# whwu95/MVFNet

Hardware: AMD Instinct MI355X
Metric: clips/sec (fwd+bwd) MVFNet-R50 8x8 224^2 (higher is better)
Workload: dtype bf16; 1 GPU; MVFNet-ResNet50 8x8, 32 clips/GPU of 8x3x224x224, bf16, train step: fwd (batch-stat BN) + loss + bwd + clip + SGD-nesterov; all through the HIP C ABI (stem + 16 bottlenecks + MVF + TSN head); clips_per_gpu=32, frames_per_clip=8, parallelism=dp1: replicas, one flat gradient all-reduce per step

## Files before the change

include/mvfnet_hip.h:

```cpp
#ifndef MVFNET_HIP_H
#define MVFNET_HIP_H

#include <stddef.h>
#include <stdint.h>

#ifdef __cplusplus
extern "C" {
#endif

#define MVF_ABI_VERSION 2

enum { MVF_OK = 0, MVF_EINVAL = -1, MVF_ESHAPE = -2, MVF_EWS = -3, MVF_EHIP = -4, MVF_EUNSUPPORTED = -5 };
enum { MVF_F32 = 0, MVF_BF16 = 1 };
enum { MVF_NCHW = 0, MVF_NHWC = 1 };
enum { MVF_VIEW_T = 1, MVF_VIEW_H = 2, MVF_VIEW_W = 4 };

int mvf_abi_version(void);
const char* mvf_last_error(void);

typedef struct {
    int32_t nt, c, h, w;
    int32_t n_segment;
    int32_t cs;
    int32_t mode;
// ... 14 lines not shown
                  const float* w_t, const float* w_h, const float* w_w,
                  const float* gamma, const float* beta, float eps, float momentum,
                  float* running_mean, float* running_var, float* save_mean, float* save_invstd,
                  void* ws, size_t ws_bytes, void* stream);

size_t mvf_bwd_workspace_bytes(const mvf_desc_t* d);
int mvf_bwd(const mvf_desc_t* d, const void* g, const void* x,
            const float* w_t, const float* w_h, const float* w_w,
            const float* gamma, const float* beta, const float* mean, const float* invstd, int training,
            void* dx, float* dw_t, float* dw_h, float* dw_w, float* dgamma, float* dbeta,
            void* ws, size_t ws_bytes, void* stream);


typedef struct {
    int32_t n, h, w;
    int32_t cin, cout;
    int32_t kh, kw, stride, pad;
    int32_t ho, wo;
    int32_t x_pix_stride;
    int32_t dtype;
    int32_t relu;
    int32_t split_c;
    int32_t x2_pix_stride;
    int32_t in_dil;
    int32_t res_c0;
    int32_t x_c0;
} mvf_conv_desc_t;

int mvf_conv2d_nhwc_fwd(const mvf_conv_desc_t* d, const void* x, const void* x2, const void* w_packed,
                        const float* bias, const void* residual, void* y, void* stream);
size_t mvf_conv2d_workspace_bytes(const mvf_conv_desc_t* d);
int mvf_conv2d_nhwc_fwd_ws(const mvf_conv_desc_t* d, const void* x, const void* x2, const void* w_packed,
                           const float* bias, const void* residual, void* y, void* ws, size_t ws_bytes, void* stream);
int mvf_conv2d_nhwc_fwd_mvf(const mvf_conv_desc_t* d, const void* x, const void* w_packed, const float* bias, const float* mvf_coef,
                            int cs, int n_segment, int act, void* y, void* ws, size_t ws_bytes, void* stream);
int mvf_conv2d_nhwc_fwd_bnapply(const mvf_conv_desc_t* d, const void* x, const void* x2, const void* w_packed, const float* bn_scale,
                                const float* bn_shift, const void* residual, const float* res_scale, const float* res_shift, void* out,
                                unsigned char* sign_bits, void* ws, size_t ws_bytes, void* stream);
int mvf_conv2d_nhwc_fwd_bnbwd_sums(const mvf_conv_desc_t* d, const void* x, const void* x2, const void* w_packed, const void* g,
                                   const unsigned char* sign_bits, const float* bn_mean, const float* bn_invstd, float* sums_part, void* ws,
                                   size_t ws_bytes, void* stream);
int mvf_conv2d_nhwc_fwd_bnbwd_apply(const mvf_conv_desc_t* d, const void* x, const void* x2, const void* w_packed, const void* g,
                                    const unsigned char* sign_bits, const float* bn_gamma, const float* bn_mean, const float* bn_invstd,
                                    const float* dgamma, const float* dbeta, void* dz, void* ws, size_t ws_bytes, void* stream);
int mvf_conv2d_nhwc_fwd_resmask(const mvf_conv_desc_t* d, const void* x, const void* x2, const void* w_packed,
                                const float* bias, const void* residual, const unsigned char* res_sign_bits, void* y,
                                void* ws, size_t ws_bytes, void* stream);
int mvf_conv2d_nhwc_fwd_resmask_gate(const mvf_conv_desc_t* d, const void* x, const void* x2, const void* w_packed, const float* bias,
                                     const void* residual, const unsigned char* res_sign_bits, const unsigned char* out_gate_bits, void* y,
                                     void* ws, size_t ws_bytes, void* stream);
int mvf_conv2d_nhwc_fwd_resmask_gate_colsums(const mvf_conv_desc_t* d, const void* x, const void* x2, const void* w_packed, const void* residual,
                                             const unsigned char* res_sign_bits, const unsigned char* out_gate_bits, void* y, float* sums_part, void* ws,
                                             size_t ws_bytes, void* stream);
int mvf_conv2d_nhwc_dgrad_bnsums(const mvf_conv_desc_t* d, const void* dz, const void* w_packed_dgrad, void* y, const void* bn_z,
                                 const float* bn_mean, const float* bn_invstd, const float* bn_scale, const float* bn_shift,
                                 float* sums_part, void* ws, size_t ws_bytes, void* stream);
int mvf_bn_bwd_finalize(const float* sums_part, int nblk, int c, float* dgamma, float* dbeta, void* stream);
int mvf_conv2d_stats_rows(const mvf_conv_desc_t* d);
int mvf_conv2d_nhwc_fwd_stats(const mvf_conv_desc_t* d, const void* x, const void* x2, const void* w_packed, void* y,
                              float* stats_part, const float* stats_shift, void* ws, size_t ws_bytes, void* stream);

enum {
    MVF_CONV_FAM_NONE = 0,
    MVF_CONV_FAM_REG = 1,
    MVF_CONV_FAM_X3 = 2,
    MVF_CONV_FAM_LDS_DMA = 3,
    MVF_CONV_FAM_T256_2B = 4,
    MVF_CONV_FAM_T256_P4 = 5,
    MVF_CONV_FAM_DBUF = 6,
    MVF_CONV_FAM_DBUF_PF2 = 7,
    MVF_CONV_FAM_STREAMK = 8,
    MVF_CONV_FAM_GENERIC = 9,
    MVF_CONV_FAM_MVF_LOADER = 10,
    MVF_CONV_FAM_STEM_DIRECT = 11,
    MVF_CONV_FAM_PW_SUMS = 12,
    MVF_CONV_FAM_C3X3_C64 = 13
};
typedef struct {
    int32_t family;
    int32_t epi_asked;
    int32_t epi_run;
    int32_t pointwise;
    int32_t buffers;
    int32_t tile_m, tile_n;
    int32_t dtype;
    int32_t k_chunks;
    int32_t half_k;
    int32_t launches;
} mvf_conv_launch_info_t;
int mvf_conv2d_last_launch(mvf_conv_launch_info_t* out);

int mvf_pack_conv_weight(const float* w_oihw, int cout, int cin, int kh, int kw, int kw_pad, int cin_pad,
                         const float* scale, void* w_packed, int dtype, void* stream);
int mvf_bn_fold(const float* gamma, const float* beta, const float* mean, const float* var, float eps, int c,
                float* scale, float* shift, void* stream);

int mvf_stem_prep(const float* x_nchw, int n, int c, int h, int w, int pad, int wp, void* out, int dtype, void* stream);

int mvf_frames_prep_u8(const unsigned char* frames_hwc, int n, int hs, int ws, const int* window, int h, int w,
                       const float* mean3, const float* std3, int to_rgb, int div_255, int pad, int wp, void* out_stem,
                       float* out_nchw, int dtype, void* stream);
int mvf_frames_resample_u8(const unsigned char* frames_hwc, int n, int hs, int ws, const int* rows, int h, int w,
                           const float* mean3, const float* std3, int to_rgb, int div_255, int pad, int wp, void* out_stem,
                           float* out_nchw, int dtype, void* stream);
int mvf_frames_resample_color_u8(const unsigned char* frames_hwc, int n, int hs, int ws, const int* rows, const float* color, int h, int w,
                                 const float* mean3, const float* std3, int to_rgb, int div_255, int pad, int wp, void* out_stem,
// ... 164 lines not shown
int mvf_conv2d_nhwc_wgrad(const mvf_conv_desc_t* d, const void* dz, const void* x, const void* x2, int kw_real,
                          int cin_real, int kw_packed, int cin_packed, float* dw_oihw, void* ws, size_t ws_bytes,
                          void* stream);
int mvf_conv2d_nhwc_wgrad_wgs(const mvf_conv_desc_t* d, const void* dz, const void* x, const void* x2, int kw_real,
                              int cin_real, int kw_packed, int cin_packed, float* dw_oihw, void* ws, size_t ws_bytes, int wgs, void* stream);
enum {
    MVF_WGRAD_FAM_NONE = 0,
    MVF_WGRAD_FAM_F32_REG = 1,
    MVF_WGRAD_FAM_F32_DMA = 2,
    MVF_WGRAD_FAM_X3 = 3,
    MVF_WGRAD_FAM_BF16_WIDEN = 4,
    MVF_WGRAD_FAM_BF16_REG = 5,
    MVF_WGRAD_FAM_BF16_DMA2 = 6,
    MVF_WGRAD_FAM_BF16_PIPE = 7,
    MVF_WGRAD_FAM_T256_2B = 8,
    MVF_WGRAD_FAM_T256_P4 = 9,
    MVF_WGRAD_FAM_C3X3_C64 = 10,
    MVF_WGRAD_FAM_STEM = 11
};
typedef struct {
    int32_t family;
    int32_t stages;
    int32_t tile_co, tile_k;
    int32_t dtype;
    int32_t nsplit;
    int32_t rows_per_split;
    int32_t xcd_rr;
    int32_t split_operand;
    int32_t gram;
    int32_t wgs_target;
    int32_t launches;
} mvf_wgrad_launch_info_t;
int mvf_conv2d_wgrad_last_launch(mvf_wgrad_launch_info_t* out);
typedef struct {
    const float* w;
    void* out;
    int cout, cin, kh, kw, kw_pad, cin_pad;
    int kind, first_block;
} mvf_pack_job_t;
int mvf_pack_conv_weights_batched(const mvf_pack_job_t* jobs_dev, int njobs, int total_blocks, int dtype, void* stream);

int mvf_pack_conv_weight_dgrad(const float* w_oihw, int cout, int cin, int kh, int kw, void* w_packed, int dtype,
                               void* stream);
int mvf_nhwc_stencil(const mvf_desc_t* d, const void* x, int x_c, void* out, int out_c, const float* w_t,
                     const float* w_h, const float* w_w, const float* scale, const float* shift, int flip,
                     const void* addend, int addend_c, const unsigned char* addend_sign_bits, void* stream);
int mvf_nhwc_stencil_gate(const mvf_desc_t* d, const void* x, int x_c, void* out, int out_c, const float* w_t,
                          const float* w_h, const float* w_w, const float* scale, const float* shift, int flip,
                          const void* addend, int addend_c, const unsigned char* addend_sign_bits,
                          const unsigned char* out_gate_bits, void* stream);
int mvf_nhwc_stencil_gate_colsums(const mvf_desc_t* d, const void* x, int x_c, void* out, int out_c, const float* w_t, const float* w_h,
                                  const float* w_w, int flip, const void* addend, int addend_c, const unsigned char* addend_sign_bits,
                                  const unsigned char* out_gate_bits, float* sums_part, void* stream);
int mvf_nhwc_stencil_stats_rows(const mvf_desc_t* d, int x_c, int out_c);
int mvf_nhwc_stencil_tile_plan(const mvf_desc_t* d, int x_c, int out_c, int* rows_per_band, int* chan_per_wg);
int mvf_nhwc_stencil_stats(const mvf_desc_t* d, const void* x, int x_c, void* out, int out_c, const float* w_t, const float* w_h,
                           const float* w_w, float* stats_part, const float* stats_shift, void* stream);
size_t mvf_nhwc_tapgrad_workspace_bytes(const mvf_desc_t* d);
int mvf_nhwc_tapgrad(const mvf_desc_t* d, const void* x, int x_c, const void* dy, int dy_c, float* dw_t, float* dw_h,
                     float* dw_w, void* ws, size_t ws_bytes, void* stream);
enum {
    MVF_STENCIL_KERNEL_NONE = 0,
    MVF_STENCIL_KERNEL_WALK1 = 1,
    MVF_STENCIL_KERNEL_WALK4 = 2,
    MVF_STENCIL_KERNEL_CHUNKED = 3,
    MVF_STENCIL_KERNEL_LDS = 4
};
enum {
    MVF_STENCIL_FLIP = 1, MVF_STENCIL_HSWISH = 2, MVF_STENCIL_ADDEND = 4, MVF_STENCIL_ADDEND_BITS = 8, MVF_STENCIL_OUT_GATE = 16,
    MVF_STENCIL_STATS = 32,
    MVF_STENCIL_TAIL_COPY = 64
};
typedef struct {
    int32_t kernel;
    int32_t dtype;
    int32_t frames_per_chunk;
    int32_t rows_per_band, chan_per_wg;
    int32_t bands;
    int32_t pixels_per_wg;
    int32_t grid_x, grid_y;
    int32_t partial_rows;
    int32_t flags;
    int32_t launches;
} mvf_stencil_launch_info_t;
int mvf_nhwc_stencil_last_launch(mvf_stencil_launch_info_t* out);
enum {
    MVF_TAPGRAD_KERNEL_NONE = 0,
    MVF_TAPGRAD_KERNEL_ROWS = 1,
    MVF_TAPGRAD_KERNEL_BANDS = 2
};
typedef struct {
    int32_t kernel;
    int32_t dtype;
    int32_t nblk;
    int32_t rows_per_blk;
    int32_t cgp;
    int32_t grid_y;
    int32_t launches;
} mvf_tapgrad_launch_info_t;
int mvf_nhwc_tapgrad_last_launch(mvf_tapgrad_launch_info_t* out);
size_t mvf_sgd_workspace_bytes(long n);
int mvf_sgd_nesterov_step(float* params, const float* grads, float* momentum_buf, long n, float grad_scale, float max_norm,
                          float lr, float momentum, float weight_decay, int first_step, float* norm_out, void* ws,
                          size_t ws_bytes, void* stream);
typedef struct mvf_sgd_segment {
    long long first;
// ... 82 lines not shown
```

mvfnet_amd/_lib.py:

```python
import ctypes as C
import os

import torch

_HERE = os.path.dirname(os.path.abspath(__file__))
LIB_PATH = os.environ.get("MVF_LIB_PATH") or os.path.join(_HERE, "libmvfnet_hip.so")

MVF_F32, MVF_BF16 = 0, 1
MVF_NCHW, MVF_NHWC = 0, 1
VIEW_T, VIEW_H, VIEW_W = 1, 2, 4
MODE_BITS = {"T": 1, "TH": 3, "THW": 7}
METRICS_ROWS, METRICS_BAD_LABEL, METRICS_NAN_ROWS, METRICS_HITS, METRICS_MAX_K, METRICS_CONFUSION = 0, 1, 2, 8, 8, 16
MULTILABEL_SLOTS, MULTILABEL_NAN_ROWS, MULTILABEL_OVERFLOW, MULTILABEL_SEEN, MULTILABEL_STATE_WORDS = 0, 1, 2, 3, 8
ERRNAMES = {-1: "MVF_EINVAL", -2: "MVF_ESHAPE", -3: "MVF_EWS", -4: "MVF_EHIP", -5: "MVF_EUNSUPPORTED"}


class MvfDesc(C.Structure):
    _fields_ = [("nt", C.c_int32), ("c", C.c_int32), ("h", C.c_int32), ("w", C.c_int32), ("n_segment", C.c_int32),
                ("cs", C.c_int32), ("mode", C.c_int32), ("layout", C.c_int32), ("dtype", C.c_int32)]


class ConvDesc(C.Structure):
    _fields_ = [("n", C.c_int32), ("h", C.c_int32), ("w", C.c_int32), ("cin", C.c_int32), ("cout", C.c_int32),
                ("kh", C.c_int32), ("kw", C.c_int32), ("stride", C.c_int32), ("pad", C.c_int32),
# ... 84 lines not shown
    _fields_ = [("ptr", C.c_void_p), ("first", C.c_long)]


def _load():
    if not os.path.exists(LIB_PATH):
        raise ImportError(
            "mvfnet_amd: %s not found. Build it with `python -m mvfnet_amd.build` (needs hipcc, "
            "--offload-arch=gfx950). There is no CPU or PyTorch fallback for the hot path." % LIB_PATH)
    lib = C.CDLL(LIB_PATH)
    vp, fp, sz, i32, f32 = C.c_void_p, C.c_void_p, C.c_size_t, C.c_int, C.c_float
    dp = C.POINTER(MvfDesc)
    lib.mvf_abi_version.restype = i32
    lib.mvf_abi_version.argtypes = []
    lib.mvf_last_error.restype = C.c_char_p
    lib.mvf_last_error.argtypes = []
    lib.mvf_fwd_infer.restype = i32
    lib.mvf_fwd_infer.argtypes = [dp, vp, vp, fp, fp, fp, fp, fp, vp]
    lib.mvf_fwd_train_workspace_bytes.restype = sz
    lib.mvf_fwd_train_workspace_bytes.argtypes = [dp]
    lib.mvf_fwd_train.restype = i32
    lib.mvf_fwd_train.argtypes = [dp, vp, vp, fp, fp, fp, fp, fp, f32, f32, fp, fp, fp, fp, vp, sz, vp]
    lib.mvf_bwd_workspace_bytes.restype = sz
    lib.mvf_bwd_workspace_bytes.argtypes = [dp]
    lib.mvf_bwd.restype = i32
    lib.mvf_bwd.argtypes = [dp, vp, vp, fp, fp, fp, fp, fp, fp, fp, i32, vp, fp, fp, fp, fp, fp, vp, sz, vp]
    lib.mvf_fwd_infer_slice.restype = i32
    lib.mvf_fwd_infer_slice.argtypes = [dp, vp, vp, fp, fp, fp, fp, fp, vp]
    cp = C.POINTER(ConvDesc)
    lib.mvf_conv2d_nhwc_fwd.restype = i32
    lib.mvf_conv2d_nhwc_fwd.argtypes = [cp, vp, vp, vp, fp, vp, vp, vp]
    lib.mvf_conv2d_workspace_bytes.restype = sz
    lib.mvf_conv2d_workspace_bytes.argtypes = [cp]
    lib.mvf_conv2d_nhwc_fwd_ws.restype = i32
    lib.mvf_conv2d_nhwc_fwd_ws.argtypes = [cp, vp, vp, vp, fp, vp, vp, vp, sz, vp]
    lib.mvf_conv2d_nhwc_dgrad_bnsums.restype = i32
    lib.mvf_conv2d_nhwc_dgrad_bnsums.argtypes = [cp, vp, vp, vp, vp, fp, fp, fp, fp, fp, vp, sz, vp]
    lib.mvf_bn_bwd_finalize.restype = i32
    lib.mvf_bn_bwd_finalize.argtypes = [fp, i32, i32, fp, fp, vp]
    lib.mvf_conv2d_nhwc_fwd_bnapply.restype = i32
    lib.mvf_conv2d_nhwc_fwd_bnapply.argtypes = [cp, vp, vp, vp, fp, fp, vp, fp, fp, vp, vp, vp, sz, vp]
    lib.mvf_conv2d_nhwc_fwd_bnbwd_sums.restype = i32
    lib.mvf_conv2d_nhwc_fwd_bnbwd_sums.argtypes = [cp, vp, vp, vp, vp, vp, fp, fp, fp, vp, sz, vp]
    lib.mvf_conv2d_nhwc_fwd_bnbwd_apply.restype = i32
    lib.mvf_conv2d_nhwc_fwd_bnbwd_apply.argtypes = [cp, vp, vp, vp, vp, vp, fp, fp, fp, fp, fp, vp, vp, sz, vp]
    lib.mvf_conv2d_nhwc_fwd_resmask.restype = i32
    lib.mvf_conv2d_nhwc_fwd_resmask.argtypes = [cp, vp, vp, vp, fp, vp, vp, vp, vp, sz, vp]
    i64_ = C.c_long
    lib.mvf_conv2d_nhwc_fwd_resmask_gate.restype = i32
    lib.mvf_conv2d_nhwc_fwd_resmask_gate.argtypes = [cp, vp, vp, vp, fp, vp, vp, vp, vp, vp, sz, vp]
    lib.mvf_conv2d_nhwc_fwd_resmask_gate_colsums.restype = i32
    lib.mvf_conv2d_nhwc_fwd_resmask_gate_colsums.argtypes = [cp, vp, vp, vp, vp, vp, vp, vp, fp, vp, sz, vp]
    lib.mvf_nhwc_stencil_gate_colsums.restype = i32
    lib.mvf_nhwc_stencil_gate_colsums.argtypes = [dp, vp, i32, vp, i32, fp, fp, fp, i32, vp, i32, vp, vp, fp, vp]
    lib.mvf_conv2d_nhwc_dgrad_bnsums_split.restype = i32
    lib.mvf_conv2d_nhwc_dgrad_bnsums_split.argtypes = [cp, vp, vp, vp, fp, vp, vp, fp, fp, fp, fp, fp, vp, sz, vp]
    lib.mvf_bn_bwd_dzfree_prep.restype = i32
    lib.mvf_bn_bwd_dzfree_prep.argtypes = [vp, i32, i32, fp, fp, fp, fp, fp, i64_, vp, fp, i32, vp]
    lib.mvf_bn_bwd_dzfree_wgrad.restype = i32
    lib.mvf_bn_bwd_dzfree_wgrad.argtypes = [fp, vp, fp, fp, fp, fp, fp, fp, fp, i64_, i32, i32, i32, vp]
    lib.mvf_bn_bwd_dzfree_sums.restype = i32
    lib.mvf_bn_bwd_dzfree_sums.argtypes = [fp, vp, i32, i32, fp, fp, fp, i32, i32, fp, i32, fp, fp, i32, vp]
    lib.mvf_nhwc_stencil_stats_rows.restype = i32
    lib.mvf_nhwc_stencil_stats_rows.argtypes = [dp, i32, i32]
    lib.mvf_nhwc_stencil_tile_plan.restype = i32
    lib.mvf_nhwc_stencil_tile_plan.argtypes = [dp, i32, i32, C.POINTER(C.c_int), C.POINTER(C.c_int)]
    lib.mvf_nhwc_stencil_stats.restype = i32
    lib.mvf_nhwc_stencil_stats.argtypes = [dp, vp, i32, vp, i32, fp, fp, fp, fp, fp, vp]
    lib.mvf_nhwc_stencil_gate.restype = i32
    lib.mvf_nhwc_stencil_gate.argtypes = [dp, vp, i32, vp, i32, fp, fp, fp, fp, fp, i32, vp, i32, vp, vp, vp]
    lib.mvf_conv2d_stats_rows.restype = i32
    lib.mvf_conv2d_stats_rows.argtypes = [cp]
    lib.mvf_conv2d_nhwc_fwd_stats.restype = i32
    lib.mvf_conv2d_nhwc_fwd_stats.argtypes = [cp, vp, vp, vp, vp, fp, fp, vp, sz, vp]
    lib.mvf_conv2d_last_launch.restype = i32
    lib.mvf_conv2d_last_launch.argtypes = [C.POINTER(ConvLaunchInfo)]
    lib.mvf_pack_conv_weight.restype = i32
    lib.mvf_pack_conv_weight.argtypes = [fp, i32, i32, i32, i32, i32, i32, fp, vp, i32, vp]
    lib.mvf_pack_conv_weights_batched.restype = i32
    lib.mvf_pack_conv_weights_batched.argtypes = [vp, i32, i32, i32, vp]
    lib.mvf_bn_fold.restype = i32
    lib.mvf_bn_fold.argtypes = [fp, fp, fp, fp, f32, i32, fp, fp, vp]
    lib.mvf_stem_prep.restype = i32
    lib.mvf_stem_prep.argtypes = [fp, i32, i32, i32, i32, i32, i32, vp, i32, vp]
    lib.mvf_frames_prep_u8.restype = i32
    lib.mvf_frames_prep_u8.argtypes = [vp, i32, i32, i32, vp, i32, i32, C.POINTER(C.c_float), C.POINTER(C.c_float),
                                       i32, i32, i32, i32, vp, vp, i32, vp]
    lib.mvf_frames_resample_u8.restype = i32
    lib.mvf_frames_resample_u8.argtypes = [vp, i32, i32, i32, vp, i32, i32, C.POINTER(C.c_float), C.POINTER(C.c_float),
                                           i32, i32, i32, i32, vp, vp, i32, vp]
    lib.mvf_frames_resample_color_u8.restype = i32
    lib.mvf_frames_resample_color_u8.argtypes = [vp, i32, i32, i32, vp, vp, i32, i32, C.POINTER(C.c_float), C.POINTER(C.c_float),
                                                 i32, i32, i32, i32, vp, vp, i32, vp]
    lib.mvf_frames_gather_resample_u8.restype = i32
    lib.mvf_frames_gather_resample_u8.argtypes = [vp, i32, i32, i32, vp, i32, vp, vp, i32, i32, C.POINTER(C.c_float), C.POINTER(C.c_float),
                                                  i32, i32, i32, i32, vp, vp, i32, vp]
    lib.mvf_frames_yuv420_gather_resample_u8.restype = i32
    lib.mvf_frames_yuv420_gather_resample_u8.argtypes = [vp, i32, i32, i32, i32, i32, i32, i32, vp, i32, vp, vp, i32, i32, C.POINTER(C.c_float),
                                                         C.POINTER(C.c_float), i32, i32, i32, i32, vp, vp, i32, vp]
    lib.mvf_frames_addressed_resample_u8.restype = i32
    lib.mvf_frames_addressed_resample_u8.argtypes = [vp, C.c_longlong, i32, i32, i32, i32, vp, vp, vp, i32, i32, C.POINTER(C.c_float), C.POINTER(C.c_float),
                                                     i32, i32, i32, i32, vp, vp, i32, vp]
    lib.mvf_maxpool3x3s2_nhwc.restype = i32
    lib.mvf_maxpool3x3s2_nhwc.argtypes = [vp, i32, i32, i32, i32, vp, i32, vp]
    lib.mvf_head_pool_fc.restype = i32
    lib.mvf_head_pool_fc.argtypes = [vp, i32, i32, i32, i32, fp, fp, i32, fp, fp, i32, vp]
    lib.mvf_average_clip.restype = i32
# ... 185 lines not shown
```

mvfnet_amd/csrc/conv_nhwc.hip:

```cpp
#include <algorithm>
#include <type_traits>
#include <stdlib.h>
#include <string.h>

#include "common.h"

namespace {

constexpr int kThreads = 256;
constexpr int kPitch = 144;
constexpr int kBM = 128;

typedef float f32x16 __attribute__((ext_vector_type(16)));
typedef short bf16x8 __attribute__((ext_vector_type(8)));

struct ConvArgs {
    const char* x;
    const char* x2;
    const char* w;
    const char* res;
    const float* bias;
    char* y;
    int N, H, W, Cin, Cout, KH, KW, stride, pad, Ho, Wo;
    int xps, split_c, x2ps, relu;
    int res_c0;
    const unsigned char* res_mask;
    const unsigned char* out_gate;
    int x_c0;
    int mask_lds;
    int prio;
    int dil;
    int pad_w;
    int w_kh0, w_kw0, w_ts, w_kwfull;
    int o_s, o_ph, o_pw, o_hfull, o_wfull;
    float* stats_part;
    int stats_rows;
    const float* stats_shift;
    const char* bn_z;
    const float *bn_mean, *bn_invstd, *bn_scale, *bn_shift;
    const float *ap_scale, *ap_shift, *ap_rscale, *ap_rshift;
    unsigned char* ap_bits;
    const float *bw_gamma, *bw_dgamma, *bw_dbeta;
    int bw_mode;
    const float* mvf_coef;
    int mvf_cs, mvf_T, mvf_act;
    unsigned fd_t_mul, fd_t_shr;
    int M;
    int cpt;
    int nchunks;
    long wK;
    int tiles_m, tiles_n;
    unsigned fd_hw_mul, fd_hw_shr, fd_w_mul, fd_w_shr;
};

template <typename ET>
struct TT;
template <>
struct TT<float> {
    static constexpr int ESZ = 4, UE = 4, CE = 32;
};
template <>
struct TT<bf16_t> {
    static constexpr int ESZ = 2, UE = 8, CE = 64;
};

thread_local mvf_conv_launch_info_t t_last_launch = {};
inline void note_launch(int family, int epi_asked, int epi_run, bool pw, int buffers, int bm, int bn, int esz, int nchunks, bool half_k = false) {
    mvf_conv_launch_info_t& r = t_last_launch;
    const int launches = r.launches + 1;
    r = mvf_conv_launch_info_t{family, epi_asked, epi_run, pw ? 1 : 0, buffers, bm, bn, esz == 4 ? MVF_F32 : MVF_BF16, nchunks, half_k ? 1 : 0, launches};
}

__device__ __forceinline__ int fd_div(int n, unsigned mul, unsigned shr) { return (int)((__umulhi((unsigned)n, mul) + (unsigned)n) >> shr); }
inline void fd_make(unsigned d, unsigned& mul, unsigned& shr) {
    unsigned l = 0;
    while ((1ull << l) < d) ++l;
    mul = (unsigned)((((1ull << l) - d) << 32) / d + 1);
    shr = l;
// ... 714 lines not shown
    }

#ifdef MVF_CONV_ABLATE
    if (a.prio & 16) return;
#endif
    if (mode == SEG_PRODUCE) {
        float* slot = sk.ws + (long)g_self * (BM * BN);
#pragma unroll
        for (int i = 0; i < TM; ++i)
#pragma unroll
            for (int j = 0; j < TN; ++j)
#pragma unroll
                for (int r = 0; r < 16; ++r) slot[((i * TN + j) * 16 + r) * NT + tid] = acc[i][j][r];
        asm volatile("s_waitcnt vmcnt(0)" ::: "memory");
        __syncthreads();
        if (tid == 0) {
            __builtin_amdgcn_fence(__ATOMIC_RELEASE, "agent");
            asm volatile("s_waitcnt vmcnt(0)" ::: "memory");
            __hip_atomic_store(sk.flags + g_self, 1u, __ATOMIC_RELAXED, __HIP_MEMORY_SCOPE_AGENT);
        }
        return;
    }
    if (mode == SEG_FINISH) {
        for (int g = g_first; g < g_self; ++g) {
            if (tid == 0) {
                unsigned spins = 0;
                while (__hip_atomic_load(sk.flags + g, __ATOMIC_RELAXED, __HIP_MEMORY_SCOPE_AGENT) == 0u) {
                    __builtin_amdgcn_s_sleep(4);
                    if (++spins > (1u << 26)) {
                        __hip_atomic_store(sk.err, 1u, __ATOMIC_RELAXED, __HIP_MEMORY_SCOPE_AGENT);
                        break;
                    }
                }
                __builtin_amdgcn_fence(__ATOMIC_ACQUIRE, "agent");
            }
            __syncthreads();
            const float* slot = sk.ws + (long)g * (BM * BN);
#pragma unroll
            for (int i = 0; i < TM; ++i)
#pragma unroll
                for (int j = 0; j < TN; ++j)
#pragma unroll
                    for (int r = 0; r < 16; ++r) acc[i][j][r] += slot[((i * TN + j) * 16 + r) * NT + tid];
        }
    }

    const bool e_bias = EPI == 0 ? a.bias != nullptr : (EPI == 4 || EPI == 5 || (EPI == 6 && a.bias != nullptr));
    const bool e_res = EPI == 0 ? a.res != nullptr : (EPI == 3 || EPI == 5 || EPI == 8 || EPI == 9 || EPI == 10 || EPI == 12);
    constexpr bool e_bw = EPI == 9 || EPI == 10;
    const bool e_relu = EPI == 0 ? a.relu != 0 : (EPI == 4 || EPI == 5);
    constexpr bool e_apply = EPI == 8;
    const bool e_stats = EPI == 0 ? a.stats_part != nullptr : (EPI == 1 || EPI == 12);
    constexpr bool e_bnb = EPI == 6;
    const bool e_scatter = (EPI == 0 || EPI == 6) && a.o_s > 0;
    constexpr int CP = BN * 4 + 16;
    constexpr int NH = (LOWK || GLDS) ? 2 : 1;
    constexpr int HR = BM / NH;
    static_assert(HR * CP <= kSmem, "C tile (or half) must fit in the A/B LDS buffers");
    static_assert(HR % 32 == 0, "half split follows the MFMA row tiles");
    constexpr int PPT = BM / kBM;
    constexpr int HPP = NH / PPT;
    static_assert(NH % PPT == 0 && HPP >= 1, "a statistics partial covers whole epilogue passes");
    constexpr int TPR = BN / 4, RPP = NT / TPR;
    const int cq = tid % TPR, r0 = tid / TPR;
    const int col = n0 + cq * 4;
    ET* y = reinterpret_cast<ET*>(a.y);
    const ET* res = reinterpret_cast<const ET*>(a.res);
    float4 bv = make_float4(0.f, 0.f, 0.f, 0.f);
    if (e_bias && col < a.Cout) bv = *reinterpret_cast<const float4*>(a.bias + col);
    float4 st1 = make_float4(0.f, 0.f, 0.f, 0.f), st2 = st1, kk = st1;
    if (e_stats && a.stats_shift && col < a.Cout) kk = *reinterpret_cast<const float4*>(a.stats_shift + col);
    float4 ap_s = st1, ap_b = st1, ap_rs = make_float4(1.f, 1.f, 1.f, 1.f), ap_rb = st1;
    if (e_apply && col < a.Cout) {
        ap_s = *reinterpret_cast<const float4*>(a.ap_scale + col); ap_b = *reinterpret_cast<const float4*>(a.ap_shift + col);
        if (a.ap_rscale) { ap_rs = *reinterpret_cast<const float4*>(a.ap_rscale + col); ap_rb = *reinterpret_cast<const float4*>(a.ap_rshift + col); }
    }
    float4 b_mu = st1, b_rs = st1, b_sc = st1, b_sh = st1;
    if (e_bnb && col < a.Cout) {
        b_mu = *reinterpret_cast<const float4*>(a.bn_mean + col); b_rs = *reinterpret_cast<const float4*>(a.bn_invstd + col);
        b_sc = *reinterpret_cast<const float4*>(a.bn_scale + col); b_sh = *reinterpret_cast<const float4*>(a.bn_shift + col);
    }
    float4 w_a = st1, w_d0 = st1, w_kx = st1;
    if (e_bw && col < a.Cout) {
        b_mu = *reinterpret_cast<const float4*>(a.bn_mean + col); b_rs = *reinterpret_cast<const float4*>(a.bn_invstd + col);
        if constexpr (EPI == 9) {
            const float inv_m = 1.0f / (float)a.M;
            const float4 ga = *reinterpret_cast<const float4*>(a.bw_gamma + col), dg = *reinterpret_cast<const float4*>(a.bw_dgamma + col),
                         db = *reinterpret_cast<const float4*>(a.bw_dbeta + col);
            w_a = make_float4(ga.x * b_rs.x, ga.y * b_rs.y, ga.z * b_rs.z, ga.w * b_rs.w);
            w_d0 = make_float4(db.x * inv_m, db.y * inv_m, db.z * inv_m, db.w * inv_m);
            w_kx = make_float4(b_rs.x * dg.x * inv_m, b_rs.y * dg.y * inv_m, b_rs.z * dg.z * inv_m, b_rs.w * dg.w * inv_m);
        }
    }
    typedef unsigned u32x2 __attribute__((ext_vector_type(2)));
    const int eimg0 = fd_div(m0, a.fd_hw_mul, a.fd_hw_shr);
    __amdgpu_buffer_rsrc_t rs_y, rs_res;
    {
        const long total = (e_scatter ? (long)a.N * a.o_hfull * a.o_wfull : (long)a.M) * a.Cout * ESZ;
        const long base = (e_scatter ? (long)eimg0 * a.o_hfull * a.o_wfull : (long)m0) * a.Cout * ESZ;
        const long left = total - base;
        const unsigned nrec = (unsigned)(left < 0x7ffffff0L ? left : 0x7ffffff0L);
        rs_y = __builtin_amdgcn_make_buffer_rsrc((void*)(a.y + base), 0, a.y ? nrec : 0u, 0x00020000);
        rs_res = __builtin_amdgcn_make_buffer_rsrc((void*)(e_res ? a.res + base : (e_bnb ? a.bn_z + base : a.y + base)), 0, nrec, 0x00020000);
    }
    const __amdgpu_buffer_rsrc_t rs_mask = __builtin_amdgcn_make_buffer_rsrc(
        (void*)(a.res_mask ? a.res_mask + (long)m0 * (a.Cout / 4) : (const unsigned char*)a.y), 0,
        (unsigned)min((long)(a.M - m0) * (a.Cout / 4), 0x7ffffff0L), 0x00020000);
    const __amdgpu_buffer_rsrc_t rs_gate = __builtin_amdgcn_make_buffer_rsrc(
        (void*)(a.out_gate ? a.out_gate + (long)m0 * (a.Cout / 4) : (const unsigned char*)a.y), 0,
        (unsigned)min((long)(a.M - m0) * (a.Cout / 4), 0x7ffffff0L), 0x00020000);
    const bool e_gate = e_res && !e_apply && !e_bw && a.out_gate != nullptr;
    (void)y; (void)res;
    constexpr int kMaskOff = HR * CP;
    constexpr int MSEG = BN / 64;
    static_assert(kMaskOff + BM * (BN / 4) <= kSmem, "mask tile must fit behind the C tile");
    const bool mask_lds = e_res && (a.res_mask || e_gate) && (a.Cout % 64 == 0) && a.mask_lds;
    if (mask_lds) {
#pragma unroll
        for (int it = tid; it < BM * MSEG; it += NT) {
            const int row = it / MSEG, seg = it - row * MSEG;
            const unsigned moff = (unsigned)(row * (a.Cout / 4) + n0 / 4 + seg * 16);
            u32x4 mv = {0x0f0f0f0fu, 0x0f0f0f0fu, 0x0f0f0f0fu, 0x0f0f0f0fu};
            if (a.res_mask) mv = __builtin_amdgcn_raw_buffer_load_b128(rs_mask, moff, 0, 0);
            if (e_gate) {
                const u32x4 gv = __builtin_amdgcn_raw_buffer_load_b128(rs_gate, moff, 0, 0);
                mv.x = (mv.x & 0x0f0f0f0fu) | ((gv.x & 0x0f0f0f0fu) << 4); mv.y = (mv.y & 0x0f0f0f0fu) | ((gv.y & 0x0f0f0f0fu) << 4);
                mv.z = (mv.z & 0x0f0f0f0fu) | ((gv.z & 0x0f0f0f0fu) << 4); mv.w = (mv.w & 0x0f0f0f0fu) | ((gv.w & 0x0f0f0f0fu) << 4);
            }
            *reinterpret_cast<uint4*>(smem + kMaskOff + row * (BN / 4) + seg * 16) = make_uint4(mv.x, mv.y, mv.z, mv.w);
        }
    }
    if constexpr (sizeof(ET) == 2 && (EPI == 1 || EPI == 2) && BM == kBM) {
        if ((a.Cout & 7) == 0) {
            constexpr int CPB = BN * 2 + 8;
            static_assert(BM * CPB <= kSmem, "bf16 C tile must fit in the A/B LDS buffers");
            constexpr int TPR8 = BN / 8, RPP8 = NT / TPR8, NPS8 = BM / RPP8;
            static_assert(2 * 2 * RPP8 * TPR8 * 16 <= kSmem, "statistics scratch");
#pragma unroll
            for (int j = 0; j < TN; ++j)
#pragma unroll
                for (int i = 0; i < TM; ++i) {
                    char* cp = smem + ((wm * TM + i) * 32 + (lane & 31)) * CPB + ((wn * TN + j) * 32 + 4 * (lane >> 5)) * 2;
#pragma unroll
                    for (int g = 0; g < 4; ++g) {
                        uint2 pk;
                        pk.x = pack_bf16x2(acc[i][j][4 * g], acc[i][j][4 * g + 1]);
                        pk.y = pack_bf16x2(acc[i][j][4 * g + 2], acc[i][j][4 * g + 3]);
                        *reinterpret_cast<uint2*>(cp + g * 16) = pk;
                    }
                }
            const int cq8 = tid % TPR8, r08 = tid / TPR8;
            const int col8 = n0 + cq8 * 8;
            const bool cok8 = col8 < a.Cout;
            float kk8[8], mu8[8], rs8[8], sc8[8], sh8[8], s1[8], s2[8];
#pragma unroll
            for (int k = 0; k < 8; ++k) { kk8[k] = mu8[k] = rs8[k] = sc8[k] = sh8[k] = s1[k] = s2[k] = 0.f; }
// ... 87 lines not shown
                    if (c4 < a.Cout && tm_i * kBM < a.M) {
                        float4 t1 = make_float4(0.f, 0.f, 0.f, 0.f), t2 = t1;
                        for (int r = 0; r < RPP8; ++r) {
                            const float4 p1 = red[((r * 2 + 0) * 2 + h) * TPR8 + cq], p2 = red[((r * 2 + 1) * 2 + h) * TPR8 + cq];
                            t1.x += p1.x; t1.y += p1.y; t1.z += p1.z; t1.w += p1.w;
                            t2.x += p2.x; t2.y += p2.y; t2.z += p2.z; t2.w += p2.w;
                        }
                        float2* p = reinterpret_cast<float2*>(a.stats_part) + (long)c4 * a.stats_rows + tm_i;
                        p[0] = make_float2(t1.x, t2.x);
                        p[a.stats_rows] = make_float2(t1.y, t2.y);
                        p[2 * (long)a.stats_rows] = make_float2(t1.z, t2.z);
                        p[3 * (long)a.stats_rows] = make_float2(t1.w, t2.w);
                    }
                }
            }
            return;
        }
    }
#pragma unroll
    for (int hf = 0; hf < NH; ++hf) {
        if (hf > 0) __syncthreads();
#pragma unroll
        for (int j = 0; j < TN; ++j)
#pragma unroll
            for (int i = 0; i < TM; ++i) {
                const int rbase = (wm * TM + i) * 32;
                if (rbase / HR != hf) continue;
                char* cp = smem + (rbase - hf * HR + (lane & 31)) * CP + ((wn * TN + j) * 32 + 4 * (lane >> 5)) * 4;
#pragma unroll
                for (int g = 0; g < 4; ++g)
                    *reinterpret_cast<float4*>(cp + g * 32) =
                        make_float4(acc[i][j][4 * g], acc[i][j][4 * g + 1], acc[i][j][4 * g + 2], acc[i][j][4 * g + 3]);
            }
        constexpr int NPS = HR / RPP;
        typedef typename std::conditional<sizeof(ET) == 2, u32x2, u32x4>::type raw_t;
        unsigned offs[NPS];
        raw_t rraw[NPS];
        {
            const int mrow0 = m0 + hf * HR + r0;
            const bool cok2 = col < a.Cout;
#pragma unroll
            for (int ps = 0; ps < NPS; ++ps) {
                const int m = mrow0 + ps * RPP;
                unsigned off;
                if (e_scatter) {
                    const int img = fd_div(m, a.fd_hw_mul, a.fd_hw_shr), rem = m - img * (a.Ho * a.Wo);
                    const int oh = fd_div(rem, a.fd_w_mul, a.fd_w_shr), ow = rem - oh * a.Wo;
                    off = (unsigned)((((img - eimg0) * a.o_hfull + oh * a.o_s + a.o_ph) * a.o_wfull + ow * a.o_s + a.o_pw) * a.Cout + col) * ESZ;
                } else {
                    off = (unsigned)((m - m0) * a.Cout + col) * ESZ;
                }
                offs[ps] = (cok2 && m < a.M) ? off : kOOB;
                if (e_res || e_bnb) {
                    const unsigned roff = (e_bnb || col >= a.res_c0) ? offs[ps] : kOOB;
                    if constexpr (sizeof(ET) == 2) rraw[ps] = __builtin_amdgcn_raw_buffer_load_b64(rs_res, roff, 0, 0);
                    else rraw[ps] = __builtin_amdgcn_raw_buffer_load_b128(rs_res, roff, 0, 0);
                }
            }
        }
        __syncthreads();
        {
            auto unpack = [](const raw_t& t) {
                if constexpr (sizeof(ET) == 2)
                    return make_float4(__uint_as_float(t.x << 16), __uint_as_float(t.x & 0xffff0000u), __uint_as_float(t.y << 16),
                                       __uint_as_float(t.y & 0xffff0000u));
                else
                    return make_float4(__uint_as_float(t.x), __uint_as_float(t.y), __uint_as_float(t.z), __uint_as_float(t.w));
            };
#pragma unroll
            for (int ps = 0; ps < NPS; ++ps) {
                const unsigned off = offs[ps];
                const bool ok = off != kOOB;
                float4 v = *reinterpret_cast<const float4*>(smem + (r0 + ps * RPP) * CP + cq * 16);
                if constexpr (e_apply) {
                    if constexpr (sizeof(ET) == 2) {
                        const unsigned p0 = pack_bf16x2(v.x, v.y), p1 = pack_bf16x2(v.z, v.w);
                        v = make_float4(__uint_as_float(p0 << 16), __uint_as_float(p0 & 0xffff0000u), __uint_as_float(p1 << 16), __uint_as_float(p1 & 0xffff0000u));
                    }
                    const float4 q = unpack(rraw[ps]);
                    float t0 = v.x * ap_s.x + ap_b.x, t1 = v.y * ap_s.y + ap_b.y, t2 = v.z * ap_s.z + ap_b.z, t3 = v.w * ap_s.w + ap_b.w;
                    t0 += q.x * ap_rs.x + ap_rb.x; t1 += q.y * ap_rs.y + ap_rb.y; t2 += q.z * ap_rs.z + ap_rb.z; t3 += q.w * ap_rs.w + ap_rb.w;
                    v = make_float4(fmaxf(t0, 0.f), fmaxf(t1, 0.f), fmaxf(t2, 0.f), fmaxf(t3, 0.f));
                    if (ok) a.ap_bits[(long)(m0 + hf * HR + r0 + ps * RPP) * (a.Cout / 4) + (col >> 2)] =
                        (unsigned char)((v.x > 0.f ? 1u : 0u) | (v.y > 0.f ? 2u : 0u) | (v.z > 0.f ? 4u : 0u) | (v.w > 0.f ? 8u : 0u));
                }
                if constexpr (e_bw) {
                    if constexpr (sizeof(ET) == 2) {
                        const unsigned p0 = pack_bf16x2(v.x, v.y), p1 = pack_bf16x2(v.z, v.w);
                        v = make_float4(__uint_as_float(p0 << 16), __uint_as_float(p0 & 0xffff0000u), __uint_as_float(p1 << 16), __uint_as_float(p1 & 0xffff0000u));
                    }
                    float4 gm = unpack(rraw[ps]);
                    const unsigned mb = mask_lds ? (unsigned)*reinterpret_cast<const unsigned char*>(smem + kMaskOff + (hf * HR + r0 + ps * RPP) * (BN / 4) + cq)
                                                 : (unsigned)__builtin_amdgcn_raw_buffer_load_b8(rs_mask, ok ? off / (4 * ESZ) : kOOB, 0, 0);
                    gm.x = (mb & 1u) ? gm.x : 0.f; gm.y = (mb & 2u) ? gm.y : 0.f; gm.z = (mb & 4u) ? gm.z : 0.f; gm.w = (mb & 8u) ? gm.w : 0.f;
                    if constexpr (EPI == 10) {
                        if (!ok) gm = make_float4(0.f, 0.f, 0.f, 0.f);
                        st1.x += gm.x; st1.y += gm.y; st1.z += gm.z; st1.w += gm.w;
                        st2.x += gm.x * ((v.x - b_mu.x) * b_rs.x); st2.y += gm.y * ((v.y - b_mu.y) * b_rs.y);
                        st2.z += gm.z * ((v.z - b_mu.z) * b_rs.z); st2.w += gm.w * ((v.w - b_mu.w) * b_rs.w);
                        continue;
                    } else {
                        v.x = w_a.x * (gm.x - w_d0.x - (v.x - b_mu.x) * w_kx.x); v.y = w_a.y * (gm.y - w_d0.y - (v.y - b_mu.y) * w_kx.y);
                        v.z = w_a.z * (gm.z - w_d0.z - (v.z - b_mu.z) * w_kx.z); v.w = w_a.w * (gm.w - w_d0.w - (v.w - b_mu.w) * w_kx.w);
                    }
                }
                if (e_bias) { v.x += bv.x; v.y += bv.y; v.z += bv.z; v.w += bv.w; }
                if (e_res && !e_apply && !e_bw) {
// ... 89 lines not shown
    SkArgs sk = {};
    conv_tile<ET, WM, WN, TM, TN, false, false, true>(a, smem, xcd_swizzle(blockIdx.x, gridDim.x), 0, a.nchunks, SEG_FULL, sk, 0, 0);
}

template <typename ET, int WM, int WN, int TM, int TN>
__global__ __launch_bounds__(kThreads) void conv_igemm_pf2_kernel(ConvArgs a) {
    extern __shared__ __attribute__((aligned(16))) char smem[];
    SkArgs sk = {};
    conv_tile<ET, WM, WN, TM, TN, false, true>(a, smem, xcd_swizzle(blockIdx.x, gridDim.x), 0, a.nchunks, SEG_FULL, sk, 0, 0);
}

template <typename ET, int WM, int WN, int TM, int TN, int EPI = 0, bool PW = false, bool MVFL = false>
__global__ __launch_bounds__(kThreads) void conv_igemm_lowk_kernel(ConvArgs a) {
    extern __shared__ __attribute__((aligned(16))) char smem[];
    SkArgs sk = {};
    conv_tile<ET, WM, WN, TM, TN, true, false, false, EPI, PW, 0, MVFL>(a, smem, xcd_swizzle(blockIdx.x, gridDim.x), 0, a.nchunks, SEG_FULL, sk, 0, 0);
}

template <int WM, int WN, int TM, int TN, int EPI = 0, bool PW = false>
__global__ __launch_bounds__(kThreads, 3) void conv_igemm_x3_kernel(ConvArgs a) {
    extern __shared__ __attribute__((aligned(16))) char smem[];
    SkArgs sk = {};
    conv_tile<float, WM, WN, TM, TN, true, false, false, EPI, PW, 0, false, false, true>(a, smem, xcd_swizzle(blockIdx.x, gridDim.x), 0, a.nchunks, SEG_FULL, sk, 0, 0);
}

template <typename ET, int WM, int WN, int TM, int TN, int EPI, int NB, bool MVFL = false, bool PW = false, bool HALFK = false>
__global__ __launch_bounds__(kThreads, (NB == 1 && !MVFL) ? 4 : 1) void conv_igemm_glds_kernel(ConvArgs a) {
    extern __shared__ __attribute__((aligned(16))) char smem[];
    SkArgs sk = {};
    conv_tile<ET, WM, WN, TM, TN, false, false, false, EPI, PW, NB, MVFL, HALFK>(a, smem, xcd_swizzle(blockIdx.x, gridDim.x), 0, a.nchunks, SEG_FULL, sk, 0, 0);
}

inline int conv_epi_spec() {
    static const int v = mvf_policy_int("conv_epi", 3);
    return v;
}

inline bool is_pointwise(const ConvArgs& a) {
    return (conv_epi_spec() & 2) && a.KH == 1 && a.KW == 1 && a.pad == 0 && a.pad_w == 0 && a.split_c == 0 && a.dil <= 1;
}

inline bool infer_like(const ConvArgs& a, int epi_spec) { return (epi_spec & 1) && a.o_s <= 0 && a.bias && a.relu && !a.stats_part; }
inline bool bnsum_epi(const ConvArgs& a) { return a.bn_z && !a.relu && !a.res; }

int conv_epi_of(const ConvArgs& a, int epi_spec) {
    const bool train_like = (epi_spec & 1) && a.o_s <= 0 && !a.bias && !a.relu;
    if (a.ap_scale) return 8;
    if (a.bw_mode == 9 || a.bw_mode == 10) return a.bw_mode;
    if (train_like && a.stats_part && !a.res && !a.bn_z) return 1;
    if (bnsum_epi(a)) return 6;
    if (train_like && !a.stats_part && !a.res) return 2;
    if (train_like && !a.stats_part && a.res) return 3;
    if (train_like && a.stats_part && a.res && a.out_gate && !a.bn_z) return 12;
    if (infer_like(a, epi_spec)) return a.res ? 5 : 4;
    return 0;
}

template <int... E, class F>
int with_epi(int epi, F&& f) {
    int rc = MVF_OK;
    const bool hit = ((epi == E ? (rc = f(std::integral_constant<int, E>{}), true) : false) || ...);
    return hit ? rc : f(std::integral_constant<int, 0>{});
}

template <typename ET, int EPI>
__global__ __launch_bounds__(512) void conv_igemm_big2_kernel(ConvArgs a) {
    extern __shared__ __attribute__((aligned(16))) char smem[];
    SkArgs sk = {};
    conv_tile<ET, 4, 2, 2, 4, false, false, false, EPI, false, 2>(a, smem, xcd_swizzle(blockIdx.x, gridDim.x), 0, a.nchunks, SEG_FULL, sk, 0, 0);
}

template <typename ET>
int launch_big2(int epi, hipStream_t st, const ConvArgs& a0) {
    ConvArgs a = a0;
    a.tiles_m = (a.M + 255) / 256;
    a.tiles_n = (a.Cout + 255) / 256;
    return with_epi<1, 2, 3, 4, 5, 6>(epi, [&](auto e) -> int {
        constexpr int lds = kGldsLds<256, 256, 2>();
        auto k = conv_igemm_big2_kernel<ET, decltype(e)::value>;
        static bool attr = false;
        if (!attr) {
            MVF_HIP_OK(hipFuncSetAttribute((const void*)k, hipFuncAttributeMaxDynamicSharedMemorySize, lds));
            attr = true;
        }
        hipLaunchKernelGGL(k, dim3(a.tiles_m * a.tiles_n), dim3(512), lds, st, a);
        note_launch(MVF_CONV_FAM_T256_2B, epi, decltype(e)::value, false, 2, 256, 256, (int)sizeof(ET), a.nchunks);
        return MVF_OK;
    });
}

template <typename ET, int EPI, bool PW>
__global__ __launch_bounds__(512) void conv_igemm_p4_kernel(ConvArgs a) {
    extern __shared__ __attribute__((aligned(16))) char smem[];
    SkArgs sk = {};
    conv_tile<ET, 2, 4, 4, 2, false, false, false, EPI, PW, 4>(a, smem, xcd_swizzle(blockIdx.x, gridDim.x), 0, a.nchunks, SEG_FULL, sk, 0, 0);
}

template <typename ET>
int launch_p4(int epi, hipStream_t st, const ConvArgs& a0) {
    if constexpr (sizeof(ET) != 2) {
        return MVF_EUNSUPPORTED;
    } else {
        ConvArgs a = a0;
        a.tiles_m = (a.M + 255) / 256;
        a.tiles_n = (a.Cout + 255) / 256;
        return with_epi<1, 2, 3, 4, 5, 6>(epi, [&](auto e) -> int {
            constexpr int EPI = decltype(e)::value, lds = kGldsLds<256, 256, 2>();
// ... 309 lines not shown
    }
    SkArgs sk;
    const long units = (long)tail * a.nchunks;
    sk.G = slots;
    sk.units_base = (int)(units / sk.G);
    sk.units_rem = (int)(units % sk.G);
    sk.tile0 = full;
    sk.ws = (float*)skh.ws;
    sk.flags = (unsigned*)((char*)skh.ws + (size_t)slots * (128 * 128 * sizeof(float)));
    sk.err = sk.flags + slots;
    MVF_HIP_OK(hipMemsetAsync(sk.flags, 0, (size_t)(slots + 1) * sizeof(unsigned), st));
    hipLaunchKernelGGL(kern_sk, dim3(sk.G), dim3(kThreads), lds, st, a, sk);
    note_launch(MVF_CONV_FAM_STREAMK, conv_epi_of(a, conv_epi_spec()), 0, false, 2, BM, BN, (int)sizeof(ET), a.nchunks);
    MVF_LAUNCH_CHECK();
    return MVF_OK;
}

}

extern "C" {

size_t mvf_conv2d_workspace_bytes(const mvf_conv_desc_t*) { return sk_ws_bytes(); }

int mvf_conv2d_last_launch(mvf_conv_launch_info_t* out) {
    MVF_REQUIRE(out, MVF_EINVAL, "conv2d_last_launch: NULL argument");
    *out = t_last_launch;
    return MVF_OK;
}

int mvf_conv2d_nhwc_fwd(const mvf_conv_desc_t* d, const void* x, const void* x2, const void* w_packed,
                        const float* bias, const void* residual, void* y, void* stream) {
    return mvf_conv2d_nhwc_fwd_ws(d, x, x2, w_packed, bias, residual, y, nullptr, 0, stream);
}

struct BnBwdSums {
    const void* z;
    const float *mean, *invstd, *scale, *shift;
};
struct MvfFuse {
    const float* coef;
    int cs, T, act;
};
struct BnBwdRecompute {
    int mode;
    const float *mean, *invstd, *gamma, *dgamma, *dbeta;
};
struct BnApply {
    const float *scale, *shift, *rscale, *rshift;
    unsigned char* bits;
};
static int conv_fwd_impl(const mvf_conv_desc_t* d, const void* x, const void* x2, const void* w_packed, const float* bias,
                         const void* residual, void* y, float* stats_part, const float* stats_shift, void* ws, size_t ws_bytes,
                         void* stream, const unsigned char* res_mask = nullptr, const BnBwdSums* bnb = nullptr, const MvfFuse* mf = nullptr,
                         const BnApply* ap = nullptr, const BnBwdRecompute* bw = nullptr, const unsigned char* out_gate = nullptr);

int mvf_conv2d_nhwc_fwd_mvf(const mvf_conv_desc_t* d, const void* x, const void* w_packed, const float* bias, const float* mvf_coef,
                            int cs, int n_segment, int act, void* y, void* ws, size_t ws_bytes, void* stream) {
    MVF_REQUIRE(d && mvf_coef && bias && cs > 0 && n_segment > 0, MVF_EINVAL, "conv2d_fwd_mvf: bad argument");
    const int ce = d->dtype == MVF_F32 ? 32 : 64;
    MVF_REQUIRE(cs % ce == 0 && cs <= d->cin && d->n % n_segment == 0 && d->ho == d->h && d->wo == d->w && d->x_pix_stride == d->cin, MVF_ESHAPE,
                "conv2d_fwd_mvf: cs=%d must be a multiple of %d (one K chunk), n a multiple of n_segment, output size = input size", cs, ce);
    MVF_REQUIRE((uintptr_t)mvf_coef % 16 == 0, MVF_EINVAL, "conv2d_fwd_mvf: mvf_coef must be 16-byte aligned");
    const MvfFuse mf = {mvf_coef, cs, n_segment, act};
    return conv_fwd_impl(d, x, nullptr, w_packed, bias, nullptr, y, nullptr, nullptr, ws, ws_bytes, stream, nullptr, nullptr, &mf);
}

int mvf_conv2d_nhwc_dgrad_bnsums(const mvf_conv_desc_t* d, const void* dz, const void* w_packed_dgrad, void* y, const void* bn_z,
                                 const float* bn_mean, const float* bn_invstd, const float* bn_scale, const float* bn_shift,
                                 float* sums_part, void* ws, size_t ws_bytes, void* stream) {
    MVF_REQUIRE(d && bn_z && bn_mean && bn_invstd && bn_scale && bn_shift && sums_part, MVF_EINVAL, "conv2d_dgrad_bnsums: NULL argument");
    const BnBwdSums b = {bn_z, bn_mean, bn_invstd, bn_scale, bn_shift};
    return conv_fwd_impl(d, dz, nullptr, w_packed_dgrad, nullptr, nullptr, y, sums_part, nullptr, ws, ws_bytes, stream, nullptr, &b);
}

int mvf_conv2d_nhwc_fwd_bnapply(const mvf_conv_desc_t* d, const void* x, const void* x2, const void* w_packed, const float* bn_scale,
                                const float* bn_shift, const void* residual, const float* res_scale, const float* res_shift, void* out,
                                unsigned char* sign_bits, void* ws, size_t ws_bytes, void* stream) {
    MVF_REQUIRE(d && bn_scale && bn_shift && residual && sign_bits, MVF_EINVAL, "conv2d_fwd_bnapply: NULL argument");
    MVF_REQUIRE((res_scale == nullptr) == (res_shift == nullptr), MVF_EINVAL, "conv2d_fwd_bnapply: res_scale / res_shift must come together");
    MVF_REQUIRE(d->in_dil <= 1 && !d->relu && d->cout % 4 == 0, MVF_EINVAL, "conv2d_fwd_bnapply: a forward launch (in_dil <= 1), relu = 0 in the descriptor");
    MVF_REQUIRE(((uintptr_t)bn_scale | (uintptr_t)bn_shift | (uintptr_t)(res_scale ? res_scale : bn_scale) | (uintptr_t)(res_shift ? res_shift : bn_shift)) % 16 == 0,
                MVF_EINVAL, "conv2d_fwd_bnapply: coefficient vectors must be 16-byte aligned");
    const BnApply ap = {bn_scale, bn_shift, res_scale, res_shift, sign_bits};
    return conv_fwd_impl(d, x, x2, w_packed, nullptr, residual, out, nullptr, nullptr, ws, ws_bytes, stream, nullptr, nullptr, nullptr, &ap);
}

int mvf_conv2d_nhwc_fwd_bnbwd_sums(const mvf_conv_desc_t* d, const void* x, const void* x2, const void* w_packed, const void* g,
                                   const unsigned char* sign_bits, const float* bn_mean, const float* bn_invstd, float* sums_part, void* ws,
                                   size_t ws_bytes, void* stream) {
    MVF_REQUIRE(d && g && sign_bits && bn_mean && bn_invstd && sums_part, MVF_EINVAL, "conv2d_fwd_bnbwd_sums: NULL argument");
    MVF_REQUIRE(d->in_dil <= 1 && !d->relu, MVF_EINVAL, "conv2d_fwd_bnbwd_sums: a forward launch (in_dil <= 1), relu = 0");
    MVF_REQUIRE(((uintptr_t)bn_mean | (uintptr_t)bn_invstd) % 16 == 0, MVF_EINVAL, "conv2d_fwd_bnbwd_sums: coefficient vectors must be 16-byte aligned");
    const BnBwdRecompute bw = {10, bn_mean, bn_invstd, nullptr, nullptr, nullptr};
    return conv_fwd_impl(d, x, x2, w_packed, nullptr, g, nullptr, sums_part, nullptr, ws, ws_bytes, stream, sign_bits, nullptr, nullptr, nullptr, &bw);
}

int mvf_conv2d_nhwc_fwd_bnbwd_apply(const mvf_conv_desc_t* d, const void* x, const void* x2, const void* w_packed, const void* g,
                                    const unsigned char* sign_bits, const float* bn_gamma, const float* bn_mean, const float* bn_invstd,
                                    const float* dgamma, const float* dbeta, void* dz, void* ws, size_t ws_bytes, void* stream) {
    MVF_REQUIRE(d && g && sign_bits && bn_gamma && bn_mean && bn_invstd && dgamma && dbeta && dz, MVF_EINVAL, "conv2d_fwd_bnbwd_apply: NULL argument");
    MVF_REQUIRE(d->in_dil <= 1 && !d->relu, MVF_EINVAL, "conv2d_fwd_bnbwd_apply: a forward launch (in_dil <= 1), relu = 0");
    MVF_REQUIRE(((uintptr_t)bn_gamma | (uintptr_t)bn_mean | (uintptr_t)bn_invstd | (uintptr_t)dgamma | (uintptr_t)dbeta) % 16 == 0, MVF_EINVAL,
                "conv2d_fwd_bnbwd_apply: coefficient vectors must be 16-byte aligned");
    const BnBwdRecompute bw = {9, bn_mean, bn_invstd, bn_gamma, dgamma, dbeta};
    return conv_fwd_impl(d, x, x2, w_packed, nullptr, g, dz, nullptr, nullptr, ws, ws_bytes, stream, sign_bits, nullptr, nullptr, nullptr, &bw);
}

int mvf_conv2d_nhwc_fwd_resmask(const mvf_conv_desc_t* d, const void* x, const void* x2, const void* w_packed, const float* bias,
                                const void* residual, const unsigned char* res_sign_bits, void* y, void* ws, size_t ws_bytes,
                                void* stream) {
    MVF_REQUIRE(!res_sign_bits || (residual && d && d->in_dil <= 1), MVF_EINVAL, "conv2d_resmask: needs a residual and a stride-1 / non-dilated launch");
    return conv_fwd_impl(d, x, x2, w_packed, bias, residual, y, nullptr, nullptr, ws, ws_bytes, stream, res_sign_bits);
}

int mvf_conv2d_nhwc_fwd_resmask_gate(const mvf_conv_desc_t* d, const void* x, const void* x2, const void* w_packed, const float* bias,
                                     const void* residual, const unsigned char* res_sign_bits, const unsigned char* out_gate_bits, void* y,
                                     void* ws, size_t ws_bytes, void* stream) {
    MVF_REQUIRE(d && residual && out_gate_bits && d->in_dil <= 1 && !d->relu, MVF_EINVAL, "conv2d_resmask_gate: needs a residual, the gate bits and a stride-1 / non-dilated launch without ReLU");
    MVF_REQUIRE(((uintptr_t)out_gate_bits | (uintptr_t)(res_sign_bits ? res_sign_bits : out_gate_bits)) % 16 == 0 || d->cout % 64 != 0, MVF_EINVAL,
                "conv2d_resmask_gate: gate byte rows must be 16-byte aligned");
    return conv_fwd_impl(d, x, x2, w_packed, bias, residual, y, nullptr, nullptr, ws, ws_bytes, stream, res_sign_bits, nullptr, nullptr, nullptr, nullptr, out_gate_bits);
}

int mvf_conv2d_nhwc_fwd_resmask_gate_colsums(const mvf_conv_desc_t* d, const void* x, const void* x2, const void* w_packed, const void* residual,
                                             const unsigned char* res_sign_bits, const unsigned char* out_gate_bits, void* y, float* sums_part, void* ws, size_t ws_bytes,
                                             void* stream) {
    MVF_REQUIRE(d && residual && out_gate_bits && sums_part && d->in_dil <= 1 && !d->relu, MVF_EINVAL,
                "conv2d_resmask_gate_colsums: needs a residual, the gate bits, a partial buffer and a stride-1 launch without ReLU");
    MVF_REQUIRE(((uintptr_t)out_gate_bits | (uintptr_t)(res_sign_bits ? res_sign_bits : out_gate_bits)) % 16 == 0 || d->cout % 64 != 0, MVF_EINVAL,
                "conv2d_resmask_gate_colsums: gate byte rows must be 16-byte aligned");
    return conv_fwd_impl(d, x, x2, w_packed, nullptr, residual, y, sums_part, nullptr, ws, ws_bytes, stream, res_sign_bits, nullptr, nullptr, nullptr, nullptr, out_gate_bits);
}

int mvf_conv2d_nhwc_dgrad_bnsums_split(const mvf_conv_desc_t* d, const void* x, const void* x2, const void* w_packed, const float* bias, void* y,
                                       const void* bn_z, const float* bn_mean, const float* bn_invstd, const float* bn_scale, const float* bn_shift,
                                       float* sums_part, void* ws, size_t ws_bytes, void* stream) {
    MVF_REQUIRE(d && bn_z && bn_mean && bn_invstd && bn_scale && bn_shift && sums_part, MVF_EINVAL, "conv2d_dgrad_bnsums_split: NULL argument");
    MVF_REQUIRE(d->in_dil <= 1 && !d->relu && d->kh == 1 && d->kw == 1 && d->stride == 1, MVF_EINVAL, "conv2d_dgrad_bnsums_split: a pointwise stride-1 launch");
    const BnBwdSums b = {bn_z, bn_mean, bn_invstd, bn_scale, bn_shift};
    return conv_fwd_impl(d, x, x2, w_packed, bias, nullptr, y, sums_part, nullptr, ws, ws_bytes, stream, nullptr, &b);
}

int mvf_conv2d_nhwc_fwd_ws(const mvf_conv_desc_t* d, const void* x, const void* x2, const void* w_packed,
                           const float* bias, const void* residual, void* y, void* ws, size_t ws_bytes, void* stream) {
    return conv_fwd_impl(d, x, x2, w_packed, bias, residual, y, nullptr, nullptr, ws, ws_bytes, stream);
}

int mvf_conv2d_stats_rows(const mvf_conv_desc_t* d) {
    if (!d || d->n <= 0 || d->ho <= 0 || d->wo <= 0) return 0;
    if (d->in_dil > 1) {
        long rows = 0;
        for (int ph = 0; ph < d->in_dil; ++ph)
            for (int pw = 0; pw < d->in_dil; ++pw) {
                const long ho = (d->ho - ph + d->in_dil - 1) / d->in_dil, wo = (d->wo - pw + d->in_dil - 1) / d->in_dil;
                if (ho > 0 && wo > 0) rows += ((long)d->n * ho * wo + kBM - 1) / kBM;
            }
        return (int)rows;
    }
    return (int)(((long)d->n * d->ho * d->wo + kBM - 1) / kBM);
}

int mvf_conv2d_nhwc_fwd_stats(const mvf_conv_desc_t* d, const void* x, const void* x2, const void* w_packed, void* y,
                              float* stats_part, const float* stats_shift, void* ws, size_t ws_bytes, void* stream) {
    MVF_REQUIRE(stats_part, MVF_EINVAL, "conv2d_fwd_stats: stats_part is NULL");
    MVF_REQUIRE(!d || d->in_dil <= 1, MVF_EINVAL, "conv2d_fwd_stats: not for data-gradient launches");
    return conv_fwd_impl(d, x, x2, w_packed, nullptr, nullptr, y, stats_part, stats_shift, ws, ws_bytes, stream);
}

static int conv_fwd_impl(const mvf_conv_desc_t* d, const void* x, const void* x2, const void* w_packed, const float* bias,
                         const void* residual, void* y, float* stats_part, const float* stats_shift, void* ws, size_t ws_bytes,
                         void* stream, const unsigned char* res_mask, const BnBwdSums* bnb, const MvfFuse* mf, const BnApply* ap, const BnBwdRecompute* bw,
                         const unsigned char* out_gate) {
    t_last_launch = mvf_conv_launch_info_t{};
    MVF_REQUIRE(d && x && w_packed && (y || (stats_part && !bnb)), MVF_EINVAL, "conv2d: NULL argument");
    MVF_REQUIRE(d->dtype == MVF_F32 || d->dtype == MVF_BF16, MVF_EINVAL, "conv2d: bad dtype %d", d->dtype);
    MVF_REQUIRE(d->n > 0 && d->h > 0 && d->w > 0 && d->cin > 0 && d->cout > 0 && d->kh > 0 && d->kw > 0 &&
                    d->stride > 0 && d->pad >= 0, MVF_ESHAPE, "conv2d: bad dims");
    const int dil = d->in_dil > 1 ? d->in_dil : 1;
    MVF_REQUIRE(dil == 1 || d->stride == 1, MVF_EINVAL, "conv2d: in_dil > 1 requires stride 1");
    const int ho = ((d->h - 1) * dil + 1 + 2 * d->pad - d->kh) / d->stride + 1 + (dil - 1), wo = ((d->w - 1) * dil + 1 + 2 * d->pad - d->kw) / d->stride + 1 + (dil - 1);
    MVF_REQUIRE(d->ho > 0 && d->wo > 0 && d->ho <= ho && d->wo <= wo, MVF_ESHAPE,
                "conv2d: ho,wo = %d,%d inconsistent with input %dx%d k%dx%d s%d p%d (max %d,%d)", d->ho, d->wo, d->h,
                d->w, d->kh, d->kw, d->stride, d->pad, ho, wo);
    const int ue = d->dtype == MVF_F32 ? 4 : 8, ce = ue * 8, esz = d->dtype == MVF_F32 ? 4 : 2;
    const bool pitch_ok = d->x_pix_stride > 0 && (d->x_pix_stride % ue == 0 ||
                          ((d->x_pix_stride * 2) % ue == 0 && d->stride % 2 == 0 && d->kw == 1 && d->pad == 0 && d->w % 2 == 0));
    MVF_REQUIRE(d->cin % ue == 0 && pitch_ok, MVF_ESHAPE,
                "conv2d: cin=%d / x_pix_stride=%d do not give 16-byte aligned K chunks (unit = %d elements)", d->cin, d->x_pix_stride, ue);
    MVF_REQUIRE(((uintptr_t)x | (uintptr_t)w_packed | (uintptr_t)(x2 ? x2 : x)) % 16 == 0, MVF_EINVAL, "conv2d: pointers must be 16-byte aligned");
    if (d->split_c) {
        MVF_REQUIRE(x2 && d->kh == 1 && d->kw == 1 && d->split_c % ce == 0 && d->split_c <= d->cin && d->x2_pix_stride % ue == 0 && d->x2_pix_stride >= d->split_c,
                    MVF_EINVAL, "conv2d: split_c=%d needs x2, a 1x1 kernel and a multiple of %d channels", d->split_c, ce);
    }
    MVF_REQUIRE(d->cout % 4 == 0 && ((uintptr_t)y | (uintptr_t)(residual ? residual : y) | (uintptr_t)(bias ? (const void*)bias : y)) % 16 == 0, MVF_ESHAPE,
                "conv2d: cout=%d must be a multiple of 4 and y/residual/bias 16-byte aligned (row-wise vector epilogue)", d->cout);
    MVF_REQUIRE((long)d->n * d->ho * d->wo < (1L << 31) && (long)d->n * d->h * d->w < (1L << 31), MVF_ESHAPE, "conv2d: too many pixels");
    ConvArgs a = {};
    a.x = (const char*)x; a.x2 = (const char*)x2; a.w = (const char*)w_packed; a.res = (const char*)residual;
    a.bias = bias; a.y = (char*)y;
    a.N = d->n; a.H = d->h; a.W = d->w; a.Cin = d->cin; a.Cout = d->cout; a.KH = d->kh; a.KW = d->kw;
    a.stride = d->stride; a.pad = d->pad; a.Ho = d->ho; a.Wo = d->wo; a.xps = d->x_pix_stride;
    a.split_c = d->split_c; a.x2ps = d->x2_pix_stride; a.relu = d->relu; a.dil = dil;
    a.res_c0 = d->res_c0 > 0 ? d->res_c0 : 0;
    a.res_mask = res_mask;
    a.out_gate = out_gate;
    MVF_REQUIRE(d->x_c0 == 0 || (d->split_c > 0 && d->x_c0 > 0 && d->x_c0 <= d->split_c && d->x_c0 % ue == 0 && d->x_pix_stride >= d->cin - d->x_c0), MVF_EINVAL,
                "conv2d: x_c0=%d needs a split operand (split_c=%d), 0 < x_c0 <= split_c, a multiple of %d, and x rows of >= cin - x_c0 channels", d->x_c0, d->split_c, ue);
    a.x_c0 = d->x_c0;
    a.mask_lds = 1;
    static const int prio_on = mvf_policy_int("conv_prio", 0);
#ifdef MVF_CONV_ABLATE
    a.prio = prio_on;
#else
    a.prio = prio_on & 1;
#endif
    a.M = d->n * d->ho * d->wo;
    a.cpt = (d->cin + ce - 1) / ce;
    a.nchunks = d->kh * d->kw * a.cpt;
    a.wK = (long)d->kh * d->kw * d->cin;
    (void)esz;
    a.pad_w = d->pad; a.w_kh0 = 0; a.w_kw0 = 0; a.w_ts = 1; a.w_kwfull = d->kw;
    a.stats_part = stats_part; a.stats_shift = stats_shift;
    a.stats_rows = stats_part ? mvf_conv2d_stats_rows(d) : 0;
    if (mf) {
        a.mvf_coef = mf->coef; a.mvf_cs = mf->cs; a.mvf_T = mf->T; a.mvf_act = mf->act;
    }
    if (bw) {
        a.bw_mode = bw->mode; a.bn_mean = bw->mean; a.bn_invstd = bw->invstd; a.bw_gamma = bw->gamma; a.bw_dgamma = bw->dgamma; a.bw_dbeta = bw->dbeta;
    }
    if (ap) {
        a.ap_scale = ap->scale; a.ap_shift = ap->shift; a.ap_rscale = ap->rscale; a.ap_rshift = ap->rshift; a.ap_bits = ap->bits;
    }
    if (bnb) {
        a.bn_z = (const char*)bnb->z; a.bn_mean = bnb->mean; a.bn_invstd = bnb->invstd; a.bn_scale = bnb->scale; a.bn_shift = bnb->shift;
    }
    hipStream_t st = (hipStream_t)stream;
    SkHost skh = {ws, ws_bytes};
    auto launch = [&](const ConvArgs& aa) -> int {
        const bool narrow = d->cout <= 64;
        if (d->dtype == MVF_F32) {
            if (narrow) return launch_conv<float, 4, 1, 1, 2>(aa, skh, st);
            return launch_conv<float, 2, 2, 2, 2>(aa, skh, st);
        }
        if (narrow) return launch_conv<bf16_t, 4, 1, 1, 2>(aa, skh, st);
        return launch_conv<bf16_t, 2, 2, 2, 2>(aa, skh, st);
    };
    if (dil == 1 && d->dtype == MVF_BF16 && d->kh == 7 && d->kw == 1 && d->cin == 32 && d->x_pix_stride == 4 && d->stride == 2 && d->pad == 0 &&
        d->cout == 64 && !d->split_c && !residual && !res_mask && !bnb && !mf && !ap && !bw && y && d->res_c0 <= 0) {
        const int epi = (stats_part && !bias && !d->relu) ? 1 : ((bias && d->relu && !stats_part) ? 4 : 0);
        if (epi) {
            StemDirectArgs s = {x, w_packed, y, bias, stats_part, stats_shift, a.stats_rows, epi, d->n, d->h, d->w, d->ho, d->wo, a.wK};
            const int rc = mvf_internal::stem_direct_launch(s, st);
            if (rc == MVF_OK) note_launch(MVF_CONV_FAM_STEM_DIRECT, epi, epi, false, 0, 0, 64, 2, a.nchunks);
            if (rc != -1) return rc;
        }
    }
    if (dil == 1 && d->dtype == MVF_BF16 && d->kh == 1 && d->kw == 1 && d->stride == 1 && d->pad == 0 && d->cin == 64 && !d->split_c && !y && stats_part &&
        !bias && !d->relu && !bnb && !mf && !ap && d->ho == d->h && d->wo == d->w) {
// ... 81 lines not shown
```

mvfnet_amd/csrc/mvf_nhwc.hip:

```cpp
#include <algorithm>

#include <stdlib.h>

#include "common.h"

namespace {

constexpr int kThreads = 256;

thread_local mvf_stencil_launch_info_t t_last_stencil = {};
thread_local mvf_tapgrad_launch_info_t t_last_tapgrad = {};

struct NhwcArgs {
    const void* x;
    void* out;
    const float* wt;
    const float* wh;
    const float* ww;
    const float* scale;
    const float* shift;
    int nt, c, h, w, T, cs, mode, n_clips;
    int cg;
    int cgp;
    int pixw;
    int bands;
    int out_c;
    int flip;
    const void* add;
    int add_c;
    const unsigned char* add_mask;
    float* stats_part;
    int rb, cw, lbands;
    unsigned fdw_mul, fdw_shr, fdrw_mul, fdrw_shr;
    const float* stats_shift;
    const unsigned char* out_gate;
};

__device__ __forceinline__ float tap3(float w0, float w1, float w2, float a, float b, float c) { return __builtin_fmaf(w2, c, __builtin_fmaf(w1, b, w0 * a)); }

template <typename ET, int VEC>
struct Vec;
template <typename ET>
struct Vec<ET, 4> {
    static __device__ __forceinline__ void load(const ET* p, float (&v)[4]) {
        float4 q = ld4(p);
        v[0] = q.x; v[1] = q.y; v[2] = q.z; v[3] = q.w;
    }
    static __device__ __forceinline__ void store(ET* p, const float (&v)[4]) { st4(p, make_float4(v[0], v[1], v[2], v[3])); }
};
template <typename ET>
struct Vec<ET, 1> {
    static __device__ __forceinline__ void load(const ET* p, float (&v)[1]) { v[0] = ldf(p); }
    static __device__ __forceinline__ void store(ET* p, const float (&v)[1]) { stf(p, v[0]); }
};

template <typename ET, int VEC>
__global__ __launch_bounds__(kThreads) void mvf_nhwc_apply(NhwcArgs a) {
    const int HW = a.h * a.w, W = a.w, H = a.h, T = a.T, C = a.c;
    const int n = blockIdx.x / a.bands, band = blockIdx.x % a.bands;
    const int cgi = blockIdx.y * a.cgp + (threadIdx.x % a.cgp);
    const int plane = threadIdx.x / a.cgp, nplanes = kThreads / a.cgp;
    if (cgi >= a.cg) return;
    const int c0 = cgi * VEC;
    const bool vh = a.mode & MVF_VIEW_H, vw = a.mode & MVF_VIEW_W;
    const bool hs = a.scale != nullptr;
    float wt[VEC][3], wh[VEC][3], ww[VEC][3], sc[VEC], sh[VEC];
#pragma unroll
    for (int i = 0; i < VEC; ++i) {
#pragma unroll
        for (int j = 0; j < 3; ++j) {
            const int js = a.flip ? 2 - j : j;
            wt[i][j] = a.wt[(c0 + i) * 3 + js];
            wh[i][j] = vh ? a.wh[(c0 + i) * 3 + js] : 0.f;
            ww[i][j] = vw ? a.ww[(c0 + i) * 3 + js] : 0.f;
        }
        sc[i] = hs ? a.scale[c0 + i] : 1.f;
        sh[i] = hs ? a.shift[c0 + i] : 0.f;
    }
    const ET* x = reinterpret_cast<const ET*>(a.x);
    ET* out = reinterpret_cast<ET*>(a.out);
    const long fstride = (long)HW * C;
    const int pend = min(HW, (band + 1) * a.pixw);
    for (int pix = band * a.pixw + plane; pix < pend; pix += nplanes) {
        const int hh = pix / W, wv = pix - hh * W;
        const long e0 = ((long)n * T * HW + pix) * C + c0;
        const long o0 = ((long)n * T * HW + pix) * a.out_c + c0;
        float prev[VEC], cur[VEC], next[VEC], up[VEC], dn[VEC], lf[VEC], rt[VEC], y[VEC];
        const int t_begin = 0, t_end = T;
        Vec<ET, VEC>::load(x + e0, cur);
#pragma unroll
        for (int i = 0; i < VEC; ++i) prev[i] = 0.f;
        const bool ok_up = vh && hh > 0, ok_dn = vh && hh < H - 1, ok_lf = vw && wv > 0, ok_rt = vw && wv < W - 1;
        const long d_up = ok_up ? -(long)W * C : 0, d_dn = ok_dn ? (long)W * C : 0, d_lf = ok_lf ? -(long)C : 0, d_rt = ok_rt ? (long)C : 0;
        for (int t = t_begin; t < t_end; ++t) {
            const ET* f = x + e0 + (long)t * fstride;
            const bool ok_nx = t + 1 < T;
            Vec<ET, VEC>::load(f + (ok_nx ? fstride : 0), next);
            Vec<ET, VEC>::load(f + d_up, up);
            Vec<ET, VEC>::load(f + d_dn, dn);
            Vec<ET, VEC>::load(f + d_lf, lf);
            Vec<ET, VEC>::load(f + d_rt, rt);
#pragma unroll
            for (int i = 0; i < VEC; ++i) {
                next[i] = ok_nx ? next[i] : 0.f;
                up[i] = ok_up ? up[i] : 0.f; dn[i] = ok_dn ? dn[i] : 0.f;
                lf[i] = ok_lf ? lf[i] : 0.f; rt[i] = ok_rt ? rt[i] : 0.f;
            }
#pragma unroll
            for (int i = 0; i < VEC; ++i) {
                float yt = tap3(wt[i][0], wt[i][1], wt[i][2], prev[i], cur[i], next[i]);
                float yh = tap3(wh[i][0], wh[i][1], wh[i][2], up[i], cur[i], dn[i]);
                float yw = tap3(ww[i][0], ww[i][1], ww[i][2], lf[i], cur[i], rt[i]);
                float v = (yt + yh) + yw;
                if (hs) {
                    float u = __builtin_fmaf(sc[i], v, sh[i]);
                    v = u * (fminf(fmaxf(u + 3.0f, 0.0f), 6.0f) / 6.0f);
                }
                y[i] = v;
            }
            if (a.add) {
                float ad[VEC];
                const long apix = ((long)n * T + t) * HW + pix;
                Vec<ET, VEC>::load(reinterpret_cast<const ET*>(a.add) + apix * a.add_c + c0, ad);
                unsigned mb = 0xfu;
                if (a.add_mask) mb = a.add_mask[apix * (a.add_c / 4) + c0 / 4] >> (c0 & 3);
#pragma unroll
                for (int i = 0; i < VEC; ++i) y[i] += ((mb >> i) & 1u) ? ad[i] : 0.f;
            }
            if (a.out_gate) {
                const unsigned gb = a.out_gate[(((long)n * T + t) * HW + pix) * (a.out_c / 4) + c0 / 4] >> (c0 & 3);
#pragma unroll
                for (int i = 0; i < VEC; ++i) y[i] = ((gb >> i) & 1u) ? y[i] : 0.f;
            }
            Vec<ET, VEC>::store(out + o0 + (long)t * HW * a.out_c, y);
#pragma unroll
            for (int i = 0; i < VEC; ++i) {
                prev[i] = cur[i];
                cur[i] = next[i];
            }
        }
    }
}

template <typename ET, int TB>
__global__ __launch_bounds__(kThreads) void mvf_nhwc_apply_chunked(NhwcArgs a) {
    constexpr int VEC = 4;
    const int HW = a.h * a.w, W = a.w, H = a.h, T = a.T, C = a.c;
    const int n = blockIdx.x / a.bands, band = blockIdx.x % a.bands;
    const int cgi = blockIdx.y * a.cgp + (threadIdx.x % a.cgp);
    const int plane = threadIdx.x / a.cgp, nplanes = kThreads / a.cgp;
    const bool active = cgi < a.cg;
    if (!active && !a.stats_part) return;
    const int c0 = active ? cgi * VEC : 0;
    const bool vh = a.mode & MVF_VIEW_H, vw = a.mode & MVF_VIEW_W;
    const bool hs = a.scale != nullptr;
    float wt[VEC][3], wh[VEC][3], ww[VEC][3], sc[VEC], sh[VEC];
    float st1[VEC], st2[VEC], kk[VEC];
#pragma unroll
    for (int i = 0; i < VEC; ++i) {
        st1[i] = st2[i] = 0.f;
        kk[i] = (a.stats_part && a.stats_shift) ? a.stats_shift[c0 + i] : 0.f;
    }
    {
        auto load12 = [&](const float* p, bool on, float (&dst)[VEC][3]) {
            float f[12];
            if (on) {
                const float4 q0 = *reinterpret_cast<const float4*>(p + c0 * 3), q1 = *reinterpret_cast<const float4*>(p + c0 * 3 + 4),
                             q2 = *reinterpret_cast<const float4*>(p + c0 * 3 + 8);
                f[0] = q0.x; f[1] = q0.y; f[2] = q0.z; f[3] = q0.w; f[4] = q1.x; f[5] = q1.y; f[6] = q1.z; f[7] = q1.w;
                f[8] = q2.x; f[9] = q2.y; f[10] = q2.z; f[11] = q2.w;
            } else {
#pragma unroll
                for (int k = 0; k < 12; ++k) f[k] = 0.f;
            }
#pragma unroll
            for (int i = 0; i < VEC; ++i) {
                dst[i][0] = a.flip ? f[i * 3 + 2] : f[i * 3];
                dst[i][1] = f[i * 3 + 1];
                dst[i][2] = a.flip ? f[i * 3] : f[i * 3 + 2];
            }
        };
        load12(a.wt, true, wt);
        load12(a.wh, vh, wh);
        load12(a.ww, vw, ww);
#pragma unroll
        for (int i = 0; i < VEC; ++i) {
            sc[i] = hs ? a.scale[c0 + i] : 1.f;
            sh[i] = hs ? a.shift[c0 + i] : 0.f;
        }
    }
    const ET* x = reinterpret_cast<const ET*>(a.x);
    ET* out = reinterpret_cast<ET*>(a.out);
    const long fstride = (long)HW * C;
    const int pend = active ? min(HW, (band + 1) * a.pixw) : 0;
    for (int pix = band * a.pixw + plane; pix < pend; pix += nplanes) {
        const int hh = pix / W, wv = pix - hh * W;
        const long e0 = ((long)n * T * HW + pix) * C + c0;
        const long o0 = ((long)n * T * HW + pix) * a.out_c + c0;
        const bool ok_up = vh && hh > 0, ok_dn = vh && hh < H - 1, ok_lf = vw && wv > 0, ok_rt = vw && wv < W - 1;
        const long d_up = ok_up ? -(long)W * C : 0, d_dn = ok_dn ? (long)W * C : 0, d_lf = ok_lf ? -(long)C : 0, d_rt = ok_rt ? (long)C : 0;
        for (int t0 = 0; t0 < T; t0 += TB) {
            float cen[TB + 2][VEC], up[TB][VEC], dn[TB][VEC], lf[TB][VEC], rt[TB][VEC], ad[TB][VEC];
            unsigned mb[TB], gb[TB];
#pragma unroll
            for (int k = 0; k < TB + 2; ++k) {
                int t = t0 - 1 + k;
                t = t < 0 ? 0 : (t > T - 1 ? T - 1 : t);
                Vec<ET, VEC>::load(x + e0 + (long)t * fstride, cen[k]);
            }
#pragma unroll
            for (int k = 0; k < TB; ++k) {
                const int t = min(t0 + k, T - 1);
                const ET* f = x + e0 + (long)t * fstride;
                Vec<ET, VEC>::load(f + d_up, up[k]);
                Vec<ET, VEC>::load(f + d_dn, dn[k]);
                Vec<ET, VEC>::load(f + d_lf, lf[k]);
                Vec<ET, VEC>::load(f + d_rt, rt[k]);
                mb[k] = 0xfu;
                gb[k] = 0xfu;
                if (a.out_gate) gb[k] = a.out_gate[(((long)n * T + t) * HW + pix) * (a.out_c / 4) + c0 / 4] >> (c0 & 3);
                if (a.add) {
                    const long apix = ((long)n * T + t) * HW + pix;
                    Vec<ET, VEC>::load(reinterpret_cast<const ET*>(a.add) + apix * a.add_c + c0, ad[k]);
                    if (a.add_mask) mb[k] = a.add_mask[apix * (a.add_c / 4) + c0 / 4] >> (c0 & 3);
                }
            }
#pragma unroll
            for (int k = 0; k < TB; ++k) {
                const int t = t0 + k;
                if (t >= T) break;
                float y[VEC];
                const bool ok_pv = t > 0, ok_nx = t + 1 < T;
#pragma unroll
                for (int i = 0; i < VEC; ++i) {
                    const float pv = ok_pv ? cen[k][i] : 0.f, cu = cen[k + 1][i], nx = ok_nx ? cen[k + 2][i] : 0.f;
                    const float u_ = ok_up ? up[k][i] : 0.f, d_ = ok_dn ? dn[k][i] : 0.f, l_ = ok_lf ? lf[k][i] : 0.f, r_ = ok_rt ? rt[k][i] : 0.f;
                    float yt = tap3(wt[i][0], wt[i][1], wt[i][2], pv, cu, nx);
                    float yh = tap3(wh[i][0], wh[i][1], wh[i][2], u_, cu, d_);
                    float yw = tap3(ww[i][0], ww[i][1], ww[i][2], l_, cu, r_);
                    float v = (yt + yh) + yw;
                    if (hs) {
                        float u = __builtin_fmaf(sc[i], v, sh[i]);
                        v = u * (fminf(fmaxf(u + 3.0f, 0.0f), 6.0f) / 6.0f);
                    }
                    if (a.add) v += ((mb[k] >> i) & 1u) ? ad[k][i] : 0.f;
                    y[i] = ((gb[k] >> i) & 1u) ? v : 0.f;
                }
                Vec<ET, VEC>::store(out + o0 + (long)t * HW * a.out_c, y);
                if (a.stats_part) {
#pragma unroll
                    for (int i = 0; i < VEC; ++i) {
                        float v = y[i];
                        if constexpr (sizeof(ET) == 2) v = bf16_to_f32(f32_to_bf16(v));
                        const float dlt = v - kk[i];
                        st1[i] += dlt;
                        st2[i] += dlt * dlt;
                    }
                }
            }
        }
    }
    if (a.stats_part) {
        __shared__ float red[kThreads * 2 * VEC];
#pragma unroll
        for (int i = 0; i < VEC; ++i) {
            red[(threadIdx.x * VEC + i) * 2] = st1[i];
            red[(threadIdx.x * VEC + i) * 2 + 1] = st2[i];
        }
        __syncthreads();
        if (plane == 0 && active) {
#pragma unroll
            for (int i = 0; i < VEC; ++i) {
                float t1 = 0.f, t2 = 0.f;
                for (int q = 0; q < nplanes; ++q) {
                    t1 += red[((q * a.cgp + (threadIdx.x % a.cgp)) * VEC + i) * 2];
                    t2 += red[((q * a.cgp + (threadIdx.x % a.cgp)) * VEC + i) * 2 + 1];
                }
                reinterpret_cast<float2*>(a.stats_part)[(long)(c0 + i) * gridDim.x + blockIdx.x] = make_float2(t1, t2);
            }
        }
    }
}

__device__ __forceinline__ int fdiv(int n, unsigned mul, unsigned shr) { return (int)((__umulhi((unsigned)n, mul) + (unsigned)n) >> shr); }
inline void fdiv_make(unsigned d, unsigned& mul, unsigned& shr) {
    unsigned l = 0;
    while ((1ull << l) < d) ++l;
    mul = (unsigned)((((1ull << l) - d) << 32) / d + 1);
    shr = l;
}

template <int TT, int CW>
__global__ __launch_bounds__(kThreads, 2) void mvf_nhwc_apply_lds(NhwcArgs a) {
    extern __shared__ __attribute__((aligned(16))) char lds_tile[];
    constexpr int VEC = 4, NG = CW / VEC, PPT = CW / 8;
    const int W = a.w, H = a.h, HW = H * W, C = a.c, RB = a.rb, RP = RB + 2;
    const int n = blockIdx.x / a.lbands, band = blockIdx.x % a.lbands;
    const int cbase = blockIdx.y * CW, h0 = band * RB;
    const int tid = threadIdx.x;
    const bf16_t* x = reinterpret_cast<const bf16_t*>(a.x);
    bf16_t* out = reinterpret_cast<bf16_t*>(a.out);
    {
        const int npieces = TT * RP * W * PPT;
        const bf16_t* clip = x + (long)n * TT * HW * C + cbase;
        const i32x4 rs = rsrc_words(clip, (unsigned)(((long)TT * HW * C - cbase) * 2));
        const unsigned lds0 = (unsigned)__builtin_amdgcn_readfirstlane((int)((unsigned)(size_t)(__attribute__((address_space(3))) char*)lds_tile + (unsigned)(tid >> 6) * 1024u));
#pragma unroll
        for (int k = 0; k < 16; ++k) {
            if (__builtin_amdgcn_readfirstlane(k * kThreads + (tid & ~63)) < npieces) {
                const int idx = tid + k * kThreads;
                const int q = idx % PPT, pw = idx / PPT;
                const int t = fdiv(pw, a.fdrw_mul, a.fdrw_shr), rem = pw - t * RP * W;
                const int r = fdiv(rem, a.fdw_mul, a.fdw_shr), w = rem - r * W;
                int h = h0 - 1 + r;
                h = h < 0 ? 0 : (h > H - 1 ? H - 1 : h);
                const unsigned voff = idx < npieces ? (unsigned)(((t * HW + h * W + w) * C + q * 8) * 2) : 0xffffffffu;
                glds16(rs, lds0 + (unsigned)(k * kThreads * 16), voff);
            }
        }
    }
    const int g = tid % NG, c0 = cbase + g * VEC;
    const bool vh = a.mode & MVF_VIEW_H, vw = a.mode & MVF_VIEW_W;
    const bool hs = a.scale != nullptr;
    float wt[VEC][3], wh[VEC][3], ww[VEC][3], sc[VEC], sh[VEC], st1[VEC], st2[VEC], kk[VEC];
    {
        auto load12 = [&](const float* p, bool on, float (&dst)[VEC][3]) {
            float f[12];
            if (on) {
                const float4 q0 = *reinterpret_cast<const float4*>(p + c0 * 3), q1 = *reinterpret_cast<const float4*>(p + c0 * 3 + 4),
                             q2 = *reinterpret_cast<const float4*>(p + c0 * 3 + 8);
                f[0] = q0.x; f[1] = q0.y; f[2] = q0.z; f[3] = q0.w; f[4] = q1.x; f[5] = q1.y; f[6] = q1.z; f[7] = q1.w;
                f[8] = q2.x; f[9] = q2.y; f[10] = q2.z; f[11] = q2.w;
            } else {
#pragma unroll
                for (int k = 0; k < 12; ++k) f[k] = 0.f;
            }
#pragma unroll
            for (int i = 0; i < VEC; ++i) {
                dst[i][0] = a.flip ? f[i * 3 + 2] : f[i * 3];
                dst[i][1] = f[i * 3 + 1];
                dst[i][2] = a.flip ? f[i * 3] : f[i * 3 + 2];
            }
        };
        load12(a.wt, true, wt);
        load12(a.wh, vh, wh);
        load12(a.ww, vw, ww);
#pragma unroll
        for (int i = 0; i < VEC; ++i) {
            sc[i] = hs ? a.scale[c0 + i] : 1.f;
            sh[i] = hs ? a.shift[c0 + i] : 0.f;
            st1[i] = st2[i] = 0.f;
            kk[i] = (a.stats_part && a.stats_shift) ? a.stats_shift[c0 + i] : 0.f;
        }
    }
    asm volatile("s_waitcnt vmcnt(0)" ::: "memory");
    __syncthreads();
    const bf16_t* tile = reinterpret_cast<const bf16_t*>(lds_tile);
    const int nitems = RB * W * NG;
    const int fs = RP * W * CW;
#pragma unroll 1
    for (int it = tid; it < nitems; it += kThreads) {
        const int p = it / NG, r = fdiv(p, a.fdw_mul, a.fdw_shr), w = p - r * W, h = h0 + r;
        if (h >= H) break;
        const long pix0 = (long)n * TT * HW + h * W + w;
        constexpr int TC = 4;
        struct Side { uint2 ad[TC]; unsigned mb[TC], gb[TC]; };
        auto load_side = [&](int tc, Side& sd) {
#pragma unroll
            for (int k = 0; k < TC; ++k) {
                const long apix = pix0 + (long)(tc + k) * HW;
                sd.mb[k] = 0xfu;
                sd.gb[k] = 0xfu;
                sd.ad[k] = make_uint2(0u, 0u);
                if (a.add) {
                    sd.ad[k] = *reinterpret_cast<const uint2*>(reinterpret_cast<const bf16_t*>(a.add) + apix * a.add_c + c0);
                    if (a.add_mask) sd.mb[k] = a.add_mask[apix * (a.add_c / 4) + c0 / 4];
                }
                if (a.out_gate) sd.gb[k] = a.out_gate[apix * (a.out_c / 4) + c0 / 4];
            }
        };
        Side sd, sn;
        load_side(0, sd);
        const bool ok_up = vh && h > 0, ok_dn = vh && h < H - 1, ok_lf = vw && w > 0, ok_rt = vw && w < W - 1;
        const bf16_t* ctr = tile + ((r + 1) * W + w) * CW + g * VEC;
        const int d_up = ok_up ? -W * CW : 0, d_dn = ok_dn ? W * CW : 0, d_lf = ok_lf ? -CW : 0, d_rt = ok_rt ? CW : 0;
        float4 prev = make_float4(0.f, 0.f, 0.f, 0.f), cur = ld4(ctr);
        const int t_end = a.T;
#pragma unroll 1
        for (int tc = 0; tc < t_end; tc += TC) {
            if (tc + TC < t_end) load_side(tc + TC, sn);
#pragma unroll
            for (int k = 0; k < TC; ++k) {
                const int t = tc + k;
                const bf16_t* f = ctr + t * fs;
                float4 next = make_float4(0.f, 0.f, 0.f, 0.f);
                if (t + 1 < t_end) next = ld4(f + fs);
                const float4 u4 = ld4(f + d_up), d4 = ld4(f + d_dn), l4 = ld4(f + d_lf), r4 = ld4(f + d_rt);
                const float pv[VEC] = {prev.x, prev.y, prev.z, prev.w}, cu[VEC] = {cur.x, cur.y, cur.z, cur.w}, nx[VEC] = {next.x, next.y, next.z, next.w};
                const float uu[VEC] = {u4.x, u4.y, u4.z, u4.w}, dd[VEC] = {d4.x, d4.y, d4.z, d4.w}, ll[VEC] = {l4.x, l4.y, l4.z, l4.w}, rr[VEC] = {r4.x, r4.y, r4.z, r4.w};
                const float av[VEC] = {__uint_as_float(sd.ad[k].x << 16), __uint_as_float(sd.ad[k].x & 0xffff0000u), __uint_as_float(sd.ad[k].y << 16),
                                       __uint_as_float(sd.ad[k].y & 0xffff0000u)};
                float y[VEC];
#pragma unroll
                for (int i = 0; i < VEC; ++i) {
                    const float u_ = ok_up ? uu[i] : 0.f, d_ = ok_dn ? dd[i] : 0.f, l_ = ok_lf ? ll[i] : 0.f, r_ = ok_rt ? rr[i] : 0.f;
                    float yt = tap3(wt[i][0], wt[i][1], wt[i][2], pv[i], cu[i], nx[i]);
                    float yh = tap3(wh[i][0], wh[i][1], wh[i][2], u_, cu[i], d_);
                    float yw = tap3(ww[i][0], ww[i][1], ww[i][2], l_, cu[i], r_);
                    float v = (yt + yh) + yw;
                    if (hs) {
                        float u = __builtin_fmaf(sc[i], v, sh[i]);
                        v = u * (fminf(fmaxf(u + 3.0f, 0.0f), 6.0f) / 6.0f);
                    }
                    if (a.add) v += ((sd.mb[k] >> i) & 1u) ? av[i] : 0.f;
                    y[i] = ((sd.gb[k] >> i) & 1u) ? v : 0.f;
                }
                st4(out + (pix0 + (long)t * HW) * a.out_c + c0, make_float4(y[0], y[1], y[2], y[3]));
                if (a.stats_part) {
#pragma unroll
                    for (int i = 0; i < VEC; ++i) {
                        const float v = bf16_to_f32(f32_to_bf16(y[i]));
                        const float dlt = v - kk[i];
                        st1[i] += dlt;
                        st2[i] += dlt * dlt;
                    }
                }
                prev = cur;
                cur = next;
            }
// ... 10 lines not shown
        }
        __syncthreads();
        if (tid < NG) {
#pragma unroll
            for (int i = 0; i < VEC; ++i) {
                float t1 = 0.f, t2 = 0.f;
#pragma unroll 4
                for (int q = 0; q < kThreads / NG; ++q) {
                    t1 += red[((q * NG + tid) * VEC + i) * 2];
                    t2 += red[((q * NG + tid) * VEC + i) * 2 + 1];
                }
                reinterpret_cast<float2*>(a.stats_part)[(long)(c0 + i) * gridDim.x + blockIdx.x] = make_float2(t1, t2);
            }
        }
    }
}

struct LdsPlan { int rb, cw, bands; size_t lds; };
static bool lds_plan(int T, int H, int W, int cs, int n_clips, LdsPlan& best) {
    static const int on = mvf_policy_int("stencil_lds", 1);
    static const int min_wg = mvf_policy_int("stencil_lds_minwg", 150);
    if (!on || (T != 4 && T != 8 && T != 16)) return false;
    auto bytes = [&](int rb, int cw) { return (((size_t)T * (rb + 2) * W * cw * 2 / 16 + 63) / 64) * 1024; };
    for (size_t budget = 65536; budget >= 32768; budget >>= 1) {
        for (int cw = 64; cw >= 16; cw >>= 1) {
            if (cs % cw) continue;
            int rb = 0;
            for (int cand = std::min(H, 8); cand >= 1; --cand)
                if (bytes(cand, cw) <= budget) { rb = cand; break; }
            if (!(rb >= 2 || (rb >= 1 && rb == H))) continue;
            const int bands = (H + rb - 1) / rb;
            rb = (H + bands - 1) / bands;
            const LdsPlan p = {rb, cw, bands, bytes(rb, cw)};
            if (p.lds < (size_t)kThreads * 4 * 2 * sizeof(float)) continue;
            if ((long)n_clips * bands * (cs / cw) >= min_wg && (budget == 65536 || cw == 64)) {
                best = p;
                return true;
            }
            break;
        }
    }
    return false;
}

static bool lds_shape_plan(const mvf_desc_t* d, int out_c, LdsPlan& lp) {
    return d->dtype == MVF_BF16 && d->cs % 16 == 0 && d->c % 8 == 0 && out_c % 4 == 0 && d->n_segment > 0 &&
           (long)d->n_segment * d->h * d->w * d->c * 2 < 0x7ffffff0L &&
           lds_plan(d->n_segment, d->h, d->w, d->cs, d->nt / d->n_segment, lp);
}

template <int TT>
static void launch_lds(const NhwcArgs& a, const LdsPlan& p, hipStream_t st) {
    dim3 grid(a.n_clips * p.bands, a.cs / p.cw);
    if (p.cw == 64) hipLaunchKernelGGL((mvf_nhwc_apply_lds<TT, 64>), grid, dim3(kThreads), p.lds, st, a);
    else if (p.cw == 32) hipLaunchKernelGGL((mvf_nhwc_apply_lds<TT, 32>), grid, dim3(kThreads), p.lds, st, a);
    else hipLaunchKernelGGL((mvf_nhwc_apply_lds<TT, 16>), grid, dim3(kThreads), p.lds, st, a);
}

template <typename ET>
__global__ void copy_tail_nhwc(const ET* src, ET* dst, long npix, int c, int cs) {
    const int tail = c - cs;
    const long total = npix * tail;
    for (long i = (long)blockIdx.x * blockDim.x + threadIdx.x; i < total; i += (long)gridDim.x * blockDim.x) {
        long p = i / tail;
        int k = (int)(i - p * tail);
        dst[p * c + cs + k] = src[p * c + cs + k];
    }
}

}

struct NhwcFlip { int flip; const void* add; int add_c; const unsigned char* add_mask; const unsigned char* out_gate; float* stats_part; const float* stats_shift; int rows_only; };
int mvf_nhwc_fwd_infer_impl2(const mvf_desc_t* d, const void* x, void* out, int out_c, const float* wt, const float* wh,
                             const float* ww, const float* scale, const float* shift, NhwcFlip fl, hipStream_t st) {
    if (!fl.rows_only) t_last_stencil = mvf_stencil_launch_info_t{};
    MVF_REQUIRE(x != out, MVF_EINVAL,
                "mvf_fwd_infer(NHWC): in-place is not supported in this layout (neighbour pixels are re-read from "
                "global memory); pass a separate out buffer");
    NhwcArgs a = {};
    a.x = x; a.out = out; a.wt = wt; a.wh = wh; a.ww = ww; a.scale = scale; a.shift = shift;
    a.nt = d->nt; a.c = d->c; a.h = d->h; a.w = d->w; a.T = d->n_segment; a.cs = d->cs; a.mode = d->mode;
    a.n_clips = d->nt / d->n_segment;
    a.out_c = out_c;
    a.flip = fl.flip;
    a.add = fl.add;
    a.add_c = fl.add_c;
    a.add_mask = fl.add_mask;
    a.out_gate = fl.out_gate;
    a.stats_part = fl.stats_part;
    a.stats_shift = fl.stats_shift;
    const int esz = d->dtype == MVF_F32 ? 4 : 2;
    const bool vec = (d->cs % 4 == 0) && (d->c % 4 == 0) && (out_c % 4 == 0) && (((uintptr_t)x | (uintptr_t)out) % (4 * esz) == 0) &&
                     (!fl.add || (fl.add_c % 4 == 0 && (uintptr_t)fl.add % (4 * esz) == 0));
    MVF_REQUIRE(!fl.out_gate || vec, MVF_EUNSUPPORTED, "nhwc_stencil: the output gate needs the 4-channel kernels (cs, pitches %% 4 == 0, aligned operands)");
    a.cg = vec ? d->cs / 4 : d->cs;
    int cgp = 1;
    while (cgp < a.cg && cgp < kThreads) cgp <<= 1;
    a.cgp = cgp;
    const int HW = d->h * d->w;
    const int nplanes = kThreads / cgp;
    int per = 4;
    while (per > 1 && (long)a.n_clips * ((HW + nplanes * per - 1) / (nplanes * per)) * ((a.cg + cgp - 1) / cgp) < 1024) per >>= 1;
    int pixw = std::max(nplanes * per, 1);
    while ((long)a.n_clips * ((HW + pixw - 1) / pixw) > 8192 && pixw < HW) pixw *= 2;
    a.pixw = std::min(pixw, HW);
    a.bands = (HW + a.pixw - 1) / a.pixw;
    dim3 grid(a.n_clips * a.bands, (a.cg + cgp - 1) / cgp, 1);
    LdsPlan lp = {};
    const bool lds_shape = (!fl.add || fl.add_c % 4 == 0) && lds_shape_plan(d, out_c, lp);
    const bool use_lds = lds_shape && vec && (uintptr_t)x % 16 == 0 && ((uintptr_t)wt | (uintptr_t)(wh ? wh : wt) | (uintptr_t)(ww ? ww : wt)) % 16 == 0;
    MVF_REQUIRE(use_lds || !lds_shape || !fl.stats_part, MVF_EINVAL, "nhwc_stencil: operands of a statistics launch must be 16-byte aligned (x, taps) / 8-byte (out, addend, bn_z)");
    if (use_lds) {
        if (fl.rows_only) return a.n_clips * lp.bands;
        a.rb = lp.rb; a.cw = lp.cw; a.lbands = lp.bands;
        fdiv_make((unsigned)d->w, a.fdw_mul, a.fdw_shr);
        fdiv_make((unsigned)((lp.rb + 2) * d->w), a.fdrw_mul, a.fdrw_shr);
        if (a.T == 4) launch_lds<4>(a, lp, st);
        else if (a.T == 8) launch_lds<8>(a, lp, st);
        else launch_lds<16>(a, lp, st);
        MVF_LAUNCH_CHECK();
    }
    if (fl.rows_only) return (int)grid.x;
    static const int chunked_env = mvf_policy_int("stencil_chunked", 1);
    const bool chunked = chunked_env != 0 && vec && ((uintptr_t)wt | (uintptr_t)(wh ? wh : wt) | (uintptr_t)(ww ? ww : wt)) % 16 == 0;
    MVF_REQUIRE(!fl.stats_part || chunked || use_lds, MVF_EUNSUPPORTED, "nhwc_stencil_stats: needs the chunked 4-channel kernel (cs, pitches %% 4 == 0, 16-byte aligned taps, policy stencil_chunked != 0) or the tiled one");
    mvf_stencil_launch_info_t rec = {};
    rec.dtype = d->dtype;
    rec.flags = (fl.flip ? MVF_STENCIL_FLIP : 0) | (scale ? MVF_STENCIL_HSWISH : 0) | (fl.add ? MVF_STENCIL_ADDEND : 0) | (fl.add_mask ? MVF_STENCIL_ADDEND_BITS : 0) |
                (fl.out_gate ? MVF_STENCIL_OUT_GATE : 0) | (fl.stats_part ? MVF_STENCIL_STATS : 0);
    if (use_lds) {
        rec.kernel = MVF_STENCIL_KERNEL_LDS;
        rec.rows_per_band = lp.rb; rec.chan_per_wg = lp.cw; rec.bands = lp.bands; rec.pixels_per_wg = lp.rb * d->w;
        rec.grid_x = a.n_clips * lp.bands; rec.grid_y = d->cs / lp.cw;
    } else {
        rec.kernel = chunked ? MVF_STENCIL_KERNEL_CHUNKED : (vec ? MVF_STENCIL_KERNEL_WALK4 : MVF_STENCIL_KERNEL_WALK1);
        rec.frames_per_chunk = chunked ? (d->dtype == MVF_F32 ? 4 : 8) : 0;
        rec.bands = a.bands; rec.pixels_per_wg = a.pixw; rec.grid_x = (int)grid.x; rec.grid_y = (int)grid.y;
    }
    rec.partial_rows = fl.stats_part ? rec.grid_x : 0;
    rec.launches = 1;
    t_last_stencil = rec;
    if (use_lds) {
    } else if (d->dtype == MVF_F32) {
        if (chunked) hipLaunchKernelGGL((mvf_nhwc_apply_chunked<float, 4>), grid, dim3(kThreads), 0, st, a);
        else if (vec) hipLaunchKernelGGL((mvf_nhwc_apply<float, 4>), grid, dim3(kThreads), 0, st, a);
        else hipLaunchKernelGGL((mvf_nhwc_apply<float, 1>), grid, dim3(kThreads), 0, st, a);
    } else {
        if (chunked) hipLaunchKernelGGL((mvf_nhwc_apply_chunked<bf16_t, 8>), grid, dim3(kThreads), 0, st, a);
        else if (vec) hipLaunchKernelGGL((mvf_nhwc_apply<bf16_t, 4>), grid, dim3(kThreads), 0, st, a);
        else hipLaunchKernelGGL((mvf_nhwc_apply<bf16_t, 1>), grid, dim3(kThreads), 0, st, a);
    }
    MVF_LAUNCH_CHECK();
    if (d->cs < d->c && out_c == d->c) {
        const long npix = (long)d->nt * HW;
        const int blocks = (int)std::min<long>((npix * (d->c - d->cs) + 255) / 256, 256L * 16);
        if (d->dtype == MVF_F32)
            hipLaunchKernelGGL(copy_tail_nhwc<float>, dim3(blocks), dim3(256), 0, st, (const float*)x, (float*)out, npix, d->c, d->cs);
        else
            hipLaunchKernelGGL(copy_tail_nhwc<bf16_t>, dim3(blocks), dim3(256), 0, st, (const bf16_t*)x, (bf16_t*)out, npix, d->c, d->cs);
        MVF_LAUNCH_CHECK();
        t_last_stencil.flags |= MVF_STENCIL_TAIL_COPY;
        t_last_stencil.launches = 2;
    }
    return MVF_OK;
}

int mvf_nhwc_fwd_infer_impl(const mvf_desc_t* d, const void* x, void* out, int out_c, const float* wt, const float* wh,
                            const float* ww, const float* scale, const float* shift, hipStream_t st) {
    NhwcFlip f = {0, nullptr, 0, nullptr, nullptr, nullptr, nullptr, 0};
    return mvf_nhwc_fwd_infer_impl2(d, x, out, out_c, wt, wh, ww, scale, shift, f, st);
}

int mvf_nhwc_fwd_infer(const mvf_desc_t* d, const void* x, void* out, const float* wt, const float* wh,
                       const float* ww, const float* scale, const float* shift, hipStream_t st) {
    return mvf_nhwc_fwd_infer_impl(d, x, out, d->c, wt, wh, ww, scale, shift, st);
}

namespace {
struct NhwcTrainWs {
    size_t y, dz, coef, bn, tap, total;
};
NhwcTrainWs nhwc_train_ws(const mvf_desc_t* d) {
    const size_t esz = d->dtype == MVF_F32 ? 4 : 2;
    const size_t m = (size_t)d->nt * d->h * d->w;
    NhwcTrainWs w;
    size_t o = 0;
    w.y = o;    o += align_up(m * d->cs * esz, 256);
    w.dz = o;   o += align_up(m * d->cs * esz, 256);
    w.coef = o; o += align_up((size_t)4 * d->cs * sizeof(float), 256);
    w.bn = o;   o += align_up(mvf_bn_workspace_bytes((long)m, d->cs), 256);
    w.tap = o;  o += align_up(mvf_nhwc_tapgrad_workspace_bytes(d), 256);
    w.total = o;
    return w;
}
__global__ void bn_coef_kernel(const float* gamma, const float* beta, const float* mean, const float* invstd, int c, float* coef) {
    const int i = blockIdx.x * blockDim.x + threadIdx.x;
    if (i >= c) return;
    const float s = gamma[i] * invstd[i];
    coef[i] = s;
    coef[c + i] = beta[i] - mean[i] * s;
    coef[2 * c + i] = 0.f;
// ... 237 lines not shown
bool tap_rows_on() {
    if (g_tap_rows < 0) {
        g_tap_rows = mvf_policy_int("tapgrad_rows", 1) != 0 ? 1 : 0;
    }
    return g_tap_rows != 0;
}

struct TapPlan { int cgp, pixw, bands, gy; };
TapPlan tap_plan(int n_clips, int hw, int cs) {
    TapPlan p;
    const int cg = cs / 4;
    int cgp = 1;
    while (cgp < cg && cgp < kThreads) cgp <<= 1;
    p.cgp = cgp;
    const int nplanes = kThreads / cgp;
    int pixw = std::max(nplanes * 8, 1);
    while ((long)n_clips * ((hw + pixw - 1) / pixw) > 2048 && pixw < hw) pixw *= 2;
    p.pixw = std::min(pixw, hw);
    p.bands = (hw + p.pixw - 1) / p.pixw;
    p.gy = (cg + cgp - 1) / cgp;
    return p;
}

}

extern "C" {

int mvf_nhwc_stencil(const mvf_desc_t* d, const void* x, int x_c, void* out, int out_c, const float* w_t, const float* w_h,
                     const float* w_w, const float* scale, const float* shift, int flip, const void* addend, int addend_c,
                     const unsigned char* addend_sign_bits, void* stream) {
    t_last_stencil = mvf_stencil_launch_info_t{};
    MVF_REQUIRE(d && x && out && w_t && x != out && x_c >= d->cs && out_c >= d->cs, MVF_EINVAL, "nhwc_stencil: bad argument");
    MVF_REQUIRE(!addend || addend_c >= d->cs, MVF_EINVAL, "nhwc_stencil: addend pitch < cs");
    MVF_REQUIRE(!addend_sign_bits || (addend && addend_c % 4 == 0), MVF_EINVAL, "nhwc_stencil: gate bits need an addend with pitch % 4 == 0");
    mvf_desc_t dd = *d;
    dd.c = x_c;
    NhwcFlip f = {flip, addend, addend_c, addend_sign_bits, nullptr, nullptr, nullptr, 0};
    return mvf_nhwc_fwd_infer_impl2(&dd, x, out, out_c, w_t, w_h, w_w, scale, shift, f, (hipStream_t)stream);
}

int mvf_nhwc_stencil_gate(const mvf_desc_t* d, const void* x, int x_c, void* out, int out_c, const float* w_t, const float* w_h,
                          const float* w_w, const float* scale, const float* shift, int flip, const void* addend, int addend_c,
                          const unsigned char* addend_sign_bits, const unsigned char* out_gate_bits, void* stream) {
    t_last_stencil = mvf_stencil_launch_info_t{};
    MVF_REQUIRE(d && x && out && w_t && x != out && x_c >= d->cs && out_c >= d->cs && out_gate_bits, MVF_EINVAL, "nhwc_stencil_gate: bad argument");
    MVF_REQUIRE(!addend || addend_c >= d->cs, MVF_EINVAL, "nhwc_stencil_gate: addend pitch < cs");
    MVF_REQUIRE(!addend_sign_bits || (addend && addend_c % 4 == 0), MVF_EINVAL, "nhwc_stencil_gate: gate bits need an addend with pitch % 4 == 0");
    mvf_desc_t dd = *d;
    dd.c = x_c;
    NhwcFlip f = {flip, addend, addend_c, addend_sign_bits, out_gate_bits, nullptr, nullptr, 0};
    return mvf_nhwc_fwd_infer_impl2(&dd, x, out, out_c, w_t, w_h, w_w, scale, shift, f, (hipStream_t)stream);
}

int mvf_nhwc_stencil_gate_colsums(const mvf_desc_t* d, const void* x, int x_c, void* out, int out_c, const float* w_t, const float* w_h,
                                  const float* w_w, int flip, const void* addend, int addend_c, const unsigned char* addend_sign_bits,
                                  const unsigned char* out_gate_bits, float* sums_part, void* stream) {
    t_last_stencil = mvf_stencil_launch_info_t{};
    MVF_REQUIRE(d && x && out && w_t && x != out && x_c >= d->cs && out_c >= d->cs && out_gate_bits && sums_part, MVF_EINVAL, "nhwc_stencil_gate_colsums: bad argument");
    MVF_REQUIRE(!addend || addend_c >= d->cs, MVF_EINVAL, "nhwc_stencil_gate_colsums: addend pitch < cs");
    MVF_REQUIRE(!addend_sign_bits || (addend && addend_c % 4 == 0), MVF_EINVAL, "nhwc_stencil_gate_colsums: gate bits need an addend with pitch % 4 == 0");
    mvf_desc_t dd = *d;
    dd.c = x_c;
    NhwcFlip f = {flip, addend, addend_c, addend_sign_bits, out_gate_bits, sums_part, nullptr, 0};
    return mvf_nhwc_fwd_infer_impl2(&dd, x, out, out_c, w_t, w_h, w_w, nullptr, nullptr, f, (hipStream_t)stream);
}

int mvf_nhwc_stencil_tile_plan(const mvf_desc_t* d, int x_c, int out_c, int* rows_per_band, int* chan_per_wg) {
    if (!d || d->cs <= 0 || d->nt <= 0 || d->n_segment <= 0) return 0;
    mvf_desc_t dd = *d;
    dd.c = x_c;
    LdsPlan lp = {};
    if (!lds_shape_plan(&dd, out_c, lp)) return 0;
    if (rows_per_band) *rows_per_band = lp.rb;
    if (chan_per_wg) *chan_per_wg = lp.cw;
    return 1;
}

int mvf_nhwc_stencil_stats_rows(const mvf_desc_t* d, int x_c, int out_c) {
    if (!d || d->cs <= 0 || d->nt <= 0) return 0;
    mvf_desc_t dd = *d;
    dd.c = x_c;
    NhwcFlip f = {0, nullptr, 0, nullptr, nullptr, nullptr, nullptr, 1};
    return mvf_nhwc_fwd_infer_impl2(&dd, (const void*)16, (void*)32, out_c, (const float*)16, (const float*)16, (const float*)16, nullptr, nullptr, f, nullptr);
}
int mvf_nhwc_stencil_stats(const mvf_desc_t* d, const void* x, int x_c, void* out, int out_c, const float* w_t, const float* w_h,
                           const float* w_w, float* stats_part, const float* stats_shift, void* stream) {
    t_last_stencil = mvf_stencil_launch_info_t{};
    MVF_REQUIRE(d && x && out && w_t && x != out && x_c >= d->cs && out_c >= d->cs && stats_part, MVF_EINVAL, "nhwc_stencil_stats: bad argument");
    mvf_desc_t dd = *d;
    dd.c = x_c;
    NhwcFlip f = {0, nullptr, 0, nullptr, nullptr, stats_part, stats_shift, 0};
    return mvf_nhwc_fwd_infer_impl2(&dd, x, out, out_c, w_t, w_h, w_w, nullptr, nullptr, f, (hipStream_t)stream);
}

size_t mvf_nhwc_tapgrad_workspace_bytes(const mvf_desc_t* d) {
    if (!d || d->cs <= 0 || d->cs % 4) return 0;
    TapPlan p = tap_plan(d->nt / d->n_segment, d->h * d->w, d->cs);
    TapRows q = tap_rows_plan((long)d->nt * d->h * d->w, d->cs);
    const size_t a = (size_t)(d->nt / d->n_segment) * p.bands * d->cs * 7 * sizeof(float), b = (size_t)q.nblk * d->cs * 7 * sizeof(float);
    return align_up(std::max(a, b), 256);
}

int mvf_nhwc_tapgrad(const mvf_desc_t* d, const void* x, int x_c, const void* dy, int dy_c, float* dw_t, float* dw_h, float* dw_w,
                     void* ws, size_t ws_bytes, void* stream) {
    t_last_tapgrad = mvf_tapgrad_launch_info_t{};
    MVF_REQUIRE(d && x && dy && dw_t && d->cs % 4 == 0 && x_c % 4 == 0 && dy_c % 4 == 0, MVF_EINVAL, "nhwc_tapgrad: bad argument (cs %% 4?)");
// ... 48 lines not shown
```

mvfnet_amd/train_engine.py:

```python
import ctypes as C
import os

import torch

from . import _lib
from ._lib import ConvDesc, MvfDesc, check, lib

F32 = _lib.MVF_F32

_ConvDescT, _MvfDescT = ConvDesc, MvfDesc
_DESC_CACHE = {}


def ConvDesc(*a):
    d = _DESC_CACHE.get(a)
    if d is None:
        d = _DESC_CACHE[a] = _ConvDescT(*a)
    return d


def MvfDesc(*a):
    k = ("mvf",) + a
    d = _DESC_CACHE.get(k)
    if d is None:
# ... 138 lines not shown
        return dza, dzb

    def backward_wgrad(self, g, g_pitch, z, m, eng, mask_mode, ymask, conv, x, x_pitch, sums_done=False):
        if not sums_done:
            self._reduce(g, g_pitch, z, m, eng, mask_mode, ymask, None)
        return self._apply_bwd_wgrad(g, g_pitch, z, m, eng, mask_mode, ymask, conv, x, x_pitch)

    def _apply_bwd_wgrad(self, g, g_pitch, z, m, eng, mask_mode, ymask, conv, x, x_pitch):
        dz = eng.buf((id(self), "dz"), z.shape, z.dtype)
        ns = lib.mvf_bn_bwd_wgrad_splits(m, self.c, conv.cin, 1, mask_mode)
        nb = lib.mvf_bn_bwd_wgrad_slab_bytes(m, self.c, conv.cin, 1, mask_mode)
        slabs = eng.buf((id(conv), "wslab"), (nb // 4,), torch.float32)
        sg, sb = (self._zero, self._zero) if self.frozen else (self.dgamma, self.dbeta)
        check(lib.mvf_bn_bwd_apply_wgrad(_p(g), g_pitch, _p(z), _p(ymask) if mask_mode == 4 else None, m, self.c, _p(self.gamma), _p(self.mean), _p(self.invstd),
                                         _p(self.scale), _p(self.shift), _p(sg), _p(sb), mask_mode, _p(dz), _p(x), x_pitch, conv.cin, _p(slabs), nb,
                                         eng.dt, _st()), "mvf_bn_bwd_apply_wgrad")
        conv.slab_reduce(slabs, ns, eng)
        return dz

    @staticmethod
    def backward_pair_wgrad(a, b, g, g_pitch, za, zb, m, eng, bits, conv_a, xa, xa_pitch, conv_b, xb, xb_pitch):
        nbw = lib.mvf_bn_workspace_bytes(m, a.c)
        ws = eng.workspace(2 * nbw)
        dza, dzb = eng.buf((id(a), "dz"), za.shape, za.dtype), eng.buf((id(b), "dz"), zb.shape, zb.dtype)
        k = conv_a.cin
        ns = lib.mvf_bn_bwd_wgrad_splits(m, a.c, k, 2, 4)
        nb = lib.mvf_bn_bwd_wgrad_slab_bytes(m, a.c, k, 2, 4)
        sa = eng.buf((id(conv_a), "wslab"), (nb // 4,), torch.float32)
        sb = eng.buf((id(conv_b), "wslab"), (nb // 4,), torch.float32) if xb is not None else None
        check(lib.mvf_bn_bwd_pair_wgrad(_p(g), g_pitch, _p(za), _p(zb), _p(bits), m, a.c, _p(a.gamma), _p(a.mean), _p(a.invstd), _p(a.dgamma), _p(a.dbeta),
                                        _p(b.gamma), _p(b.mean), _p(b.invstd), _p(b.dgamma), _p(b.dbeta), _p(dza), _p(dzb), _p(xa), xa_pitch,
                                        _p(xb), xb_pitch, k, _p(sa), _p(sb), nb, _p(ws), ws.numel(), eng.dt, _st()), "mvf_bn_bwd_pair_wgrad")
        conv_a.slab_reduce(sa, ns, eng)
        if xb is not None:
            conv_b.slab_reduce(sb, ns, eng)
        return dza, dzb

    def _reduce(self, g, g_pitch, z, m, eng, mask_mode, ymask, gm_out):
        ws = eng.workspace(lib.mvf_bn_workspace_bytes(m, self.c))
        check(lib.mvf_bn_bwd_reduce(_p(g), g_pitch, _p(z), _p(ymask), m, self.c, _p(self.mean), _p(self.invstd), _p(self.scale),
                                    _p(self.shift), mask_mode, _p(gm_out), _p(self.dgamma), _p(self.dbeta), _p(ws), ws.numel(), eng.dt, _st()),
              "mvf_bn_bwd_reduce")

    def _apply_bwd(self, g, g_pitch, z, m, eng, mask_mode, ymask, gm_out):
        src, pitch, mode = (gm_out, self.c, 0) if gm_out is not None else (g, g_pitch, mask_mode)
        dz = eng.buf((id(self), "dz"), z.shape, z.dtype)
        sg, sb = (self._zero, self._zero) if self.frozen else (self.dgamma, self.dbeta)
        check(lib.mvf_bn_bwd_apply_masked(_p(src), pitch, _p(z), _p(ymask) if mode in (1, 4) else None, m, self.c, _p(self.gamma), _p(self.mean),
                                          _p(self.invstd), _p(self.scale), _p(self.shift), _p(sg), _p(sb), mode, _p(dz), eng.dt,
                                          _st()), "mvf_bn_bwd_apply")
        return dz


class _TConv(object):

    def __init__(self, conv, eng, stem=False):
        self.eng = eng
        self.w = conv.weight
        self.dw = eng.grad_of(conv.weight)
        self.cout, self.cin, self.kh, self.kw = conv.weight.shape
        self.stride, self.pad = conv.stride[0], conv.padding[0]
        self.stem = stem
        dev = conv.weight.device
        td = eng.tdtype
        if stem:
            self.wp = torch.empty(self.cout, self.kh, 8, 4, device=dev, dtype=td)
            self.wd = None
        else:
            same = self.kh == 1 and self.kw == 1 and td == torch.float32
            self.wp = self.w if same else torch.empty(self.cout, self.kh, self.kw, self.cin, device=dev, dtype=td)
            self.wd = torch.empty(self.cin, self.kh, self.kw, self.cout, device=dev, dtype=td)

    def pack(self, need_dgrad=True):
        if self.stem:
            check(lib.mvf_pack_conv_weight(_p(self.w), self.cout, self.cin, self.kh, self.kw, 8, 4, None, _p(self.wp), self.eng.dt, _st()), "pack")
            return
        if self.wp is not self.w:
            check(lib.mvf_pack_conv_weight(_p(self.w), self.cout, self.cin, self.kh, self.kw, self.kw, self.cin, None, _p(self.wp), self.eng.dt, _st()), "pack")
        if need_dgrad:
            self.pack_dgrad()

    def pack_jobs(self):
        if self.stem:
            return (self.w, self.wp, self.cout, self.cin, self.kh, self.kw, 8, 4, 0), None
        fwd = None if self.wp is self.w else (self.w, self.wp, self.cout, self.cin, self.kh, self.kw, self.kw, self.cin, 0)
        return fwd, (self.w, self.wd, self.cout, self.cin, self.kh, self.kw, self.kw, self.cin, 1)

    def pack_dgrad(self):
        if not self.stem:
            check(lib.mvf_pack_conv_weight_dgrad(_p(self.w), self.cout, self.cin, self.kh, self.kw, _p(self.wd), self.eng.dt, _st()), "pack_dgrad")

    def desc(self, n, h, w, ho, wo, x_pitch, split_c=0):
        if self.stem:
            return ConvDesc(n, h, w, 32, self.cout, self.kh, 1, 2, 0, ho, wo, 4, self.eng.dt, 0, 0, 0, 0)
        return ConvDesc(n, h, w, self.cin, self.cout, self.kh, self.kw, self.stride, self.pad, ho, wo, x_pitch, self.eng.dt, 0, split_c, split_c, 0)

    def out_hw(self, h, w):
        return (h + 2 * self.pad - self.kh) // self.stride + 1, (w + 2 * self.pad - self.kw) // self.stride + 1

    def forward(self, x, n, h, w, x_pitch=None, x2=None, split_c=0, ho=None, wo=None, bn=None, store=True):
        if ho is None:
            ho, wo = self.out_hw(h, w)
        d = self.desc(n, h, w, ho, wo, x_pitch or self.cin, split_c)
        z = self.eng.buf((id(self), "z"), (n * ho * wo, self.cout)) if store else None
        ws = _conv_ws(x.device)
        if bn is None or not self.eng.fuse_stats or bn.frozen:
            self.launch_fwd(d, x, x2, z, ws, None, None)
            if bn is not None:
                bn.stats(z, n * ho * wo, self.eng)
            return z, ho, wo
        rows = _stats_rows(d)
        part = self.eng.buf((id(self), "part"), (rows, self.cout, 2), torch.float32)
        self.launch_fwd(d, x, x2, z, ws, part, bn.mod.running_mean)
        bn.finalize(part, rows, n * ho * wo)
        return z, ho, wo
# ... 72 lines not shown
                                              _p(rbn.scale if rbn else None), _p(rbn.shift if rbn else None), _p(out), _p(bits),
                                              _p(ws), ws.numel(), _st()), "conv fwd + bn apply")

    def launch_fwd(self, d, x, x2, z, ws, part, shift):
        if part is None:
            check(lib.mvf_conv2d_nhwc_fwd_ws(C.byref(d), _p(x), _p(x2), _p(self.wp), None, None, _p(z), _p(ws), ws.numel(), _st()), "conv fwd")
        else:
            check(lib.mvf_conv2d_nhwc_fwd_stats(C.byref(d), _p(x), _p(x2), _p(self.wp), _p(z), _p(part), _p(shift), _p(ws), ws.numel(), _st()),
                  "conv fwd+stats")

    def wgrad(self, dz, x, n, h, w, ho, wo, eng, x_pitch=None, x2=None, split_c=0, on_main=False):
        d = self.desc(n, h, w, ho, wo, x_pitch or self.cin, split_c)
        kwr, cinr, kwp, cinp = (self.kw, self.cin, 8, 4) if self.stem else (self.kw, self.cin, self.kw, self.cin)
        nbytes = lib.mvf_conv2d_wgrad_workspace_bytes(C.byref(d))
        side = None if on_main else eng.side_stream()
        if side is None:
            ws = eng.workspace(nbytes)
            check(lib.mvf_conv2d_nhwc_wgrad(C.byref(d), _p(dz), _p(x), _p(x2), kwr, cinr, kwp, cinp, _p(self.dw), _p(ws), ws.numel(), _st()), "conv wgrad")
            return
        ws = eng.workspace(nbytes, side=True)

        def launch():
            check(lib.mvf_conv2d_nhwc_wgrad(C.byref(d), _p(dz), _p(x), _p(x2), kwr, cinr, kwp, cinp, _p(self.dw), _p(ws), ws.numel(), _st()), "conv wgrad")
        eng.on_side(launch)

    def fuses_wgrad(self, eng, m, c, mask_mode, nbn=1):
        return (eng.tdtype == torch.bfloat16 and self.kh == 1 and self.kw == 1 and self.stride == 1 and not self.stem and c == self.cout and
                lib.mvf_bn_bwd_wgrad_splits(m, c, self.cin, nbn, mask_mode) > 0)

    def slab_reduce(self, slabs, ns, eng):
        def launch():
            check(lib.mvf_wgrad_slab_reduce(_p(slabs), ns, self.cout, self.cin, _p(self.dw), _st()), "wgrad slab reduce")
        if eng.side_stream() is None:
            launch()
        else:
            eng.on_side(launch)

    def dgrad_bnsums(self, dz, n, ho, wo, h, w, bn, z):
        d = ConvDesc(n, ho, wo, self.cout, self.cin, self.kh, self.kw, 1, self.kh - 1 - self.pad, h, w, self.cout, self.eng.dt, 0, 0, 0,
                     self.stride if self.stride > 1 else 0, 0)
        dx = self.eng.buf((id(self), "dx"), (n * h * w, self.cin))
        ws = _conv_ws(dz.device)
        rows = _stats_rows(d)
        part = self.eng.buf((id(self), "bnsums"), (rows, self.cin, 2), torch.float32)
        self.launch_dgrad_bnsums(d, dz, dx, z, bn, part, ws)
        check(lib.mvf_bn_bwd_finalize(_p(part), rows, self.cin, _p(bn.dgamma), _p(bn.dbeta), _st()), "bn bwd finalize")
        return dx

    def launch_dgrad_bnsums(self, d, dz, dx, z, bn, part, ws):
        check(lib.mvf_conv2d_nhwc_dgrad_bnsums(C.byref(d), _p(dz), _p(self.wd), _p(dx), _p(z), _p(bn.mean), _p(bn.invstd), _p(bn.scale), _p(bn.shift),
                                               _p(part), _p(ws), ws.numel(), _st()), "conv dgrad+bn sums")

    def dgrad(self, dz, n, ho, wo, h, w, residual=None, res_c0=0, res_bits=None, out_gate=None, gsum=None):
        d = ConvDesc(n, ho, wo, self.cout, self.cin, self.kh, self.kw, 1, self.kh - 1 - self.pad, h, w, self.cout, self.eng.dt, 0, 0, 0,
                     self.stride if self.stride > 1 else 0, res_c0)
        dx = self.eng.buf((id(self), "dx"), (n * h * w, self.cin))
        ws = _conv_ws(dz.device)
        if out_gate is not None and gsum is not None:
            bn = gsum["bn"]
            rows = _stats_rows(d)
            part = self.eng.buf((id(bn), "gsum_conv"), (self.cin, rows, 2), torch.float32)
            check(lib.mvf_conv2d_nhwc_fwd_resmask_gate_colsums(C.byref(d), _p(dz), None, _p(self.wd), _p(residual), _p(res_bits), _p(out_gate), _p(dx), _p(part), _p(ws),
                                                               ws.numel(), _st()), "conv dgrad (gated output + column sums)")
            bn._s1 = [None, 0, res_c0, part, rows]
        elif out_gate is not None:
            check(lib.mvf_conv2d_nhwc_fwd_resmask_gate(C.byref(d), _p(dz), None, _p(self.wd), None, _p(residual), _p(res_bits), _p(out_gate), _p(dx), _p(ws),
                                                       ws.numel(), _st()), "conv dgrad (gated output)")
        else:
            check(lib.mvf_conv2d_nhwc_fwd_resmask(C.byref(d), _p(dz), None, _p(self.wd), None, _p(residual), _p(res_bits), _p(dx), _p(ws), ws.numel(),
                                                  _st()), "conv dgrad")
        return dx

    def dzfree_ok(self, m):
        return (self.eng.tdtype == torch.bfloat16 and self.kh == 1 and self.kw == 1 and self.stride == 1 and not self.stem and
                self.cout % 256 == 0 and self.cin % 64 == 0 and self.cout <= 4096 and m * (self.cout + self.cin) * 2 < 0x7ffffff0)

    def dzfree_dgrad(self, gm, a_in, bn, n, h, w, bn_in, z_in, frozen_zero=None):
        eng = self.eng
        c, k, m = self.cout, self.cin, n * h * w
        bd = eng.buf((id(self), "dzfree_w"), (k, c + k))
        bias = eng.buf((id(self), "dzfree_b"), (k,), torch.float32)
        sg, sb = (frozen_zero, frozen_zero) if frozen_zero is not None else (bn.dgamma, bn.dbeta)
        check(lib.mvf_bn_bwd_dzfree_prep(_p(self.wd), c, k, _p(bn.gamma), _p(bn.mean), _p(bn.invstd), _p(sg), _p(sb), m, _p(bd), _p(bias), eng.dt, _st()),
              "bn backward without dz: operands")
        d = ConvDesc(n, h, w, c + k, k, 1, 1, 1, 0, h, w, k, eng.dt, 0, c, c, 0, 0, c)
        dx = eng.buf((id(self), "dx"), (m, k))
        ws = _conv_ws(gm.device)
        rows = _stats_rows(d)
        part = eng.buf((id(self), "bnsums"), (rows, k, 2), torch.float32)
        self.launch_dzfree_dgrad(d, a_in, gm, bd, bias, dx, z_in, bn_in, part, ws)
        check(lib.mvf_bn_bwd_finalize(_p(part), rows, k, _p(bn_in.dgamma), _p(bn_in.dbeta), _st()), "bn bwd finalize")
        return dx

    def launch_dzfree_dgrad(self, d, a_in, gm, bd, bias, dx, z_in, bn_in, part, ws):
        check(lib.mvf_conv2d_nhwc_dgrad_bnsums_split(C.byref(d), _p(a_in), _p(gm), _p(bd), _p(bias), _p(dx), _p(z_in), _p(bn_in.mean), _p(bn_in.invstd),
                                                     _p(bn_in.scale), _p(bn_in.shift), _p(part), _p(ws), ws.numel(), _st()), "conv dgrad on [gm | a] + bn sums")

    def dzfree_q_sums(self, gm, a_in, bn, n, h, w, eng):
        c, k = self.cout, self.cin
        d = self.desc(n, h, w, h, w, k, 0)
        ws = eng.workspace(lib.mvf_conv2d_wgrad_workspace_bytes(C.byref(d)))
        self.launch_q(d, gm, a_in, ws, eng.dzfree_q_wgs)
        lo, rows_lo, c_split, hi, rows_hi = bn._s1
        assert c_split == 0 or lo is not None, "the MVF slice's column sums are missing"
        check(lib.mvf_bn_bwd_dzfree_sums(_p(self.dw), _p(self.wp), c, k, _p(bn.mean), _p(bn.invstd), _p(lo), rows_lo, c_split, _p(hi), rows_hi, _p(bn.dgamma),
                                         _p(bn.dbeta), eng.dt, _st()), "bn backward sums from the weight-gradient GEMM")
        bn._s1 = None

    def launch_q(self, d, gm, a_in, ws, wgs):
        check(lib.mvf_conv2d_nhwc_wgrad_wgs(C.byref(d), _p(gm), _p(a_in), None, self.kw, self.cin, self.kw, self.cin, _p(self.dw), _p(ws), ws.numel(), wgs, _st()),
# ... 69 lines not shown
        self.bn = _BN(mvf.bn, eng, "mvf.bn") if self.use_hs else None
        dev = mvf.shift_conv.weight.device
        self.tmp_h = torch.empty(cs, 3, device=dev) if self.dwh is None else None
        self.tmp_w = torch.empty(cs, 3, device=dev) if self.dww is None else None

    def desc(self, nt, h, w, c):
        return MvfDesc(nt, c, h, w, self.T, self.cs, self.mode, _lib.MVF_NHWC, self.eng.dt)

    def forward(self, x, nt, h, w, c, eng):
        m = nt * h * w
        d = self.desc(nt, h, w, c)
        y = self.eng.buf((id(self), "y"), (m, self.cs))
        if self.use_hs and eng.fuse_mvf_stats and eng.fuse_stats and not self.bn.frozen and self.cs % 4 == 0:
            rows = lib.mvf_nhwc_stencil_stats_rows(C.byref(d), c, self.cs)
            part = self.eng.buf((id(self), "part"), (self.cs, rows, 2), torch.float32)
            self.launch_stencil_stats(d, x, c, y, part)
            self.bn.finalize(part, rows, m)
            return y, self.bn.apply(y, m, 2)
        self.launch_stencil(d, x, c, y, self.cs, 0, None, 0, None)
        if not self.use_hs:
            return y, y
        self.bn.stats(y, m, eng)
        return y, self.bn.apply(y, m, 2)

    def launch_stencil_stats(self, d, x, c, y, part):
        check(lib.mvf_nhwc_stencil_stats(C.byref(d), _p(x), c, _p(y), self.cs, _p(self.wt), _p(self.wh), _p(self.ww), _p(part), _p(self.bn.mod.running_mean),
                                         _st()), "mvf stencil + statistics")

    def backward(self, dxp, x, y, nt, h, w, c, eng, addend=None, addend_bits=None, out_gate=None, gsum=None):
        m = nt * h * w
        d = self.desc(nt, h, w, c)
        if self.use_hs:
            dy = self.bn.backward(dxp, c, y, m, eng, 3)
        else:
            dy = dxp[:, : self.cs].contiguous()
        nbytes = lib.mvf_nhwc_tapgrad_workspace_bytes(C.byref(d))
        dwh = self.dwh if self.dwh is not None else self.tmp_h
        dww = self.dww if self.dww is not None else self.tmp_w
        side = eng.side_stream() if (self.use_hs and not self.share) else None
        if side is None:
            ws = eng.workspace(nbytes)
            check(lib.mvf_nhwc_tapgrad(C.byref(d), _p(x), c, _p(dy), self.cs, _p(self.dwt), _p(dwh), _p(dww), _p(ws), ws.numel(), _st()), "mvf tapgrad")
            if self.share:
                self.dwt.view(self.cs, 3).add_(dwh.view(self.cs, 3) if self.mode & 2 else 0).add_(dww.view(self.cs, 3) if self.mode & 4 else 0)
        else:
            ws = eng.workspace(nbytes, side=True)

            def launch():
                check(lib.mvf_nhwc_tapgrad(C.byref(d), _p(x), c, _p(dy), self.cs, _p(self.dwt), _p(dwh), _p(dww), _p(ws), ws.numel(), _st()), "mvf tapgrad")
            eng.on_side(launch)
        self.launch_stencil(d, dy, self.cs, dxp, c, 1, addend, c if addend is not None else 0, addend_bits, out_gate, gsum)

    def launch_stencil(self, d, src, src_c, dst, dst_c, flip, addend, addend_c, addend_bits, out_gate=None, gsum=None):
        if out_gate is not None and gsum is not None:
            bn = gsum["bn"]
            rows = lib.mvf_nhwc_stencil_stats_rows(C.byref(d), src_c, dst_c)
            part = self.eng.buf((id(bn), "gsum_mvf"), (self.cs, rows, 2), torch.float32)
            check(lib.mvf_nhwc_stencil_gate_colsums(C.byref(d), _p(src), src_c, _p(dst), dst_c, _p(self.wt), _p(self.wh), _p(self.ww), flip, _p(addend), addend_c,
                                                    _p(addend_bits), _p(out_gate), _p(part), _st()), "mvf stencil (gated output + column sums)")
            bn._s1[0], bn._s1[1] = part, rows
            return
        if out_gate is not None:
            check(lib.mvf_nhwc_stencil_gate(C.byref(d), _p(src), src_c, _p(dst), dst_c, _p(self.wt), _p(self.wh), _p(self.ww), None, None, flip,
                                            _p(addend), addend_c, _p(addend_bits), _p(out_gate), _st()), "mvf stencil (gated output)")
            return
        check(lib.mvf_nhwc_stencil(C.byref(d), _p(src), src_c, _p(dst), dst_c, _p(self.wt), _p(self.wh), _p(self.ww), None, None, flip,
                                   _p(addend), addend_c, _p(addend_bits), _st()), "mvf stencil")


class _TBlock(object):
    def __init__(self, blk, eng):
        from .modules.MVF import MVF
        c1 = blk.conv1
        self.mvf = None
        if isinstance(c1, MVF):
            if c1.num_shift_channel:
                self.mvf = _TMvf(c1, eng)
            c1 = c1.net
        self.c1, self.b1 = _TConv(c1, eng), _BN(blk.bn1, eng, "bn1")
        self.c2, self.b2 = _TConv(blk.conv2, eng), _BN(blk.bn2, eng, "bn2")
        self.c3, self.b3 = _TConv(blk.conv3, eng), _BN(blk.bn3, eng, "bn3")
        self.cd = self.bd = None
        if blk.downsample is not None:
            self.cd, self.bd = _TConv(blk.downsample[0], eng), _BN(blk.downsample[1], eng, "down")
        self.split_ok = self.mvf is not None and self.mvf.cs % (32 if eng.tdtype == torch.float32 else 64) == 0

    def convs(self):
        return [c for c in (self.c1, self.c2, self.c3, self.cd) if c is not None]

    def fuse_apply(self, eng):
        f = eng.fuse_bn3_apply
        return f == 2 or (f == 1 and self.c3.cin <= 128)

    def z3_free(self, eng, m2=None):
        m2 = m2 or (1 << 16)
        if self.cd is not None:
            return self.z3_free_ds(eng, m2)
        if not (eng.z3_free and self.fuse_apply(eng) and eng.fuse_stats and not self.b3.frozen):
            return False
        if self.q_z3_free(eng, m2):
            return True
        if (eng.fuse_bnwg & 8) and eng.tdtype == torch.bfloat16 and lib.mvf_bn_bwd_wgrad_splits(m2, self.c3.cout, self.c3.cin, 1, 4) > 0:
            return False
        return eng.z3_free == 2 or self.c3.cin <= 64

    def z3_free_ds(self, eng, m2=1 << 16):
# ... 140 lines not shown
            if g_gated:
                gm = g
                if sums_done == "s1":
                    self.c3.dzfree_q_sums(gm, s["a2"], b3, nt, ho, wo, eng)
                    q_done = True
                elif not sums_done:
                    b3._reduce(gm, self.c3.cout, s["z3"], m2, eng, 0, None, None)
            else:
                assert s["z3"] is not None
                gm = eng.buf((id(b3), "gm"), s["z3"].shape, s["z3"].dtype)
                b3._reduce(g, self.c3.cout, s["z3"], m2, eng, 4, bits, gm)
            fz = b3._zero if b3.frozen else None
            da2 = self.c3.dzfree_dgrad(gm, s["a2"], b3, nt, ho, wo, self.b2, s["z2"], frozen_zero=fz)
            self.c3.dzfree_wgrad(gm, s["a2"], b3, nt, ho, wo, eng, frozen_zero=fz, q_done=q_done, gram_done=bool(s.get("gram")))
            dz3, w3_done = None, True
            del gm
        elif (eng.fuse_bnwg & 1) and self.c3.fuses_wgrad(eng, m2, self.c3.cout, 4):
            dz3 = self.b3.backward_wgrad(g, self.c3.cout, s["z3"], m2, eng, 4, bits, self.c3, s["a2"], self.c3.cin)
            w3_done = True
        else:
            dz3 = self.b3.backward(g, self.c3.cout, s["z3"], m2, eng, 4, ymask=bits)
        eng.issue_marked()
        fuse = eng.fuse_bn_bwd_sums
        if dz3 is None:
            pass
        elif fuse:
            da2 = self.c3.dgrad_bnsums(dz3, nt, ho, wo, ho, wo, self.b2, s["z2"])
        else:
            da2 = self.c3.dgrad(dz3, nt, ho, wo, ho, wo)
        if not w3_done:
            self.c3.wgrad(dz3, s["a2"], nt, ho, wo, ho, wo, eng)
        del dz3
        dz2 = self.b2.backward(da2, self.c2.cout, s["z2"], m2, eng, 2, sums_done=fuse)
        del da2
        fuse1 = fuse and (self.c2.stride == 1 or eng.fuse_bn_bwd_strided)
        if fuse1:
            da1 = self.c2.dgrad_bnsums(dz2, nt, ho, wo, h, w, self.b1, s["z1"])
        else:
            da1 = self.c2.dgrad(dz2, nt, ho, wo, h, w)
        self.c2.wgrad(dz2, s["a1"], nt, h, w, ho, wo, eng)
        del dz2
        w1_done = (eng.fuse_bnwg & 4) and self.mvf is None and self.c1.fuses_wgrad(eng, m, self.c1.cout, 2)
        if w1_done:
            dz1 = self.b1.backward_wgrad(da1, self.c1.cout, s["z1"], m, eng, 2, None, self.c1, s["x"], c, sums_done=fuse1)
        else:
            dz1 = self.b1.backward(da1, self.c1.cout, s["z1"], m, eng, 2, sums_done=fuse1)
        del da1
        resid, rbits = (g, None) if g_gated else (g, bits)
        if resid_ds is not None:
            resid, rbits = resid_ds, None
        elif self.cd is not None:
            if dzd is None:
                dzd = self.bd.backward(g, self.cd.cout, s["zd"], m2, eng, 4, ymask=bits)
            resid, rbits = self.cd.dgrad(dzd, nt, ho, wo, h, w), None
            if not wd_done:
                self.cd.wgrad(dzd, s["x"], nt, h, w, ho, wo, eng, x_pitch=c)
            del dzd
        if self.mvf is None:
            dx = self.c1.dgrad(dz1, nt, h, w, h, w, residual=resid, res_bits=rbits, out_gate=out_gate, gsum=gsum)
            self.gated_out, self.sums_out = out_gate is not None, (gsum["sums"] if gsum is not None else False)
            if not w1_done:
                self.c1.wgrad(dz1, s["x"], nt, h, w, h, w, eng, x_pitch=c)
        else:
            fuse = self.mvf.cs % 4 == 0
            og = out_gate if fuse else None
            gs = gsum if fuse else None
            dxp = self.c1.dgrad(dz1, nt, h, w, h, w, residual=resid if fuse else None, res_c0=self.mvf.cs, res_bits=rbits if fuse else None, out_gate=og, gsum=gs)
            self.gated_out, self.sums_out = og is not None, (gs["sums"] if gs is not None else False)
            if self.split_ok:
                self.c1.wgrad(dz1, s["x"], nt, h, w, h, w, eng, x_pitch=c, x2=s["o"], split_c=self.mvf.cs)
            else:
                self.c1.wgrad(dz1, s["xin"], nt, h, w, h, w, eng, x_pitch=c)
            self.mvf.backward(dxp, s["x"], s["y"], nt, h, w, c, eng, addend=resid if fuse else None, addend_bits=rbits if fuse else None, out_gate=og, gsum=gs)
            if not fuse:
                if rbits is not None:
                    resid = resid * (s["out"] > 0).to(resid.dtype)
                dx = eng.add(dxp, resid, key=id(self))
            else:
                dx = dxp
        if eng.keep_io:
            self.io = dict(x=s["x"], out=s["out"], g=g, dx=dx, h=h, w=w, c=c, ho=ho, wo=wo, g_gated=g_gated, dx_gated=self.gated_out)
        self.saved = None
        eng.flush_side(late=True)
        return dx


class _StatTable(object):

    def __init__(self, eng, bns):
        names = {id(m_): n_ for n_, m_ in eng.model.named_modules()}
        segs, self.keys, self.slices, first = [], [], [], 0
        for bn in bns:
            for attr in ("running_mean", "running_var"):
                t = getattr(bn.mod, attr)
                segs.append(_lib.StatSegment(t.data_ptr(), first))
                self.keys.append("%s.%s" % (names[id(bn.mod)], attr))
                self.slices.append((first, t.numel(), tuple(t.shape)))
                first += t.numel()
        self.bns, self.nseg, self.n = list(bns), len(segs), first
        arr = (_lib.StatSegment * len(segs))(*segs)
        self.dev = torch.frombuffer(bytearray(bytes(arr)), dtype=torch.uint8).to(eng.device)
        self.acc = torch.zeros(first, dtype=torch.float64, device=eng.device)
        self.shadow = torch.empty(first, dtype=torch.float32, device=eng.device)

    def accumulate(self):
        check(lib.mvf_bn_stats_accumulate(_p(self.dev), self.nseg, self.n, _p(self.acc), _st()), "bn stats accumulate")
# ... 57 lines not shown
    def grad_of(self, p):
        return self._grad_view[id(p)]

    def buf(self, key, shape, dtype=None):
        dt = dtype or self.tdtype
        shape = tuple(shape)
        k = (key, shape, dt)
        step = getattr(self, "forward_count", None)
        if step is not None:
            last = self._last_shape.get((key, dt))
            if last is not None and last[0] == step and last[1] != shape:
                raise RuntimeError("engine buffer %r requested with shapes %s and %s inside one step: they would share storage" % (key, last[1], shape))
            self._last_shape[(key, dt)] = (step, shape)
        t = self._bufs.get(k)
        if t is None:
            n = 1
            for v in shape:
                n *= int(v)
            ck = (key, dt)
            flat = self._caps.get(ck)
            if flat is None or flat.numel() < n:
                if flat is not None:
                    self._side_keep.append(flat)
                    self._storage_epoch += 1
                    for kk in [kk for kk in self._bufs if kk[0] == key and kk[2] == dt]:
                        del self._bufs[kk]
                flat = torch.empty(max(n, 1), device=self.device, dtype=dt)
                self._caps[ck] = flat
            t = flat[:n].view(shape)
            self._bufs[k] = t
        return t

    def workspace(self, nbytes, side=False):
        key = "_ws_side" if side else "_ws"
        ws = getattr(self, key, None)
        if ws is None or ws.numel() < nbytes:
            if ws is not None:
                self._storage_epoch += 1
            ws = torch.empty(max(int(nbytes), 1 << 20), dtype=torch.uint8, device=self.device)
            setattr(self, key, ws)
        return ws

    _storage_epoch = 0

    overlap_wgrad = True
    keep_io = False
    fuse_stats = True
    overlap_downsample = _policy("side_downsample", 1) != 0
    z3_free = _policy("z3_free", 1)
    fuse_bn3_apply = _policy("fuse_bn3_apply", 1)
    fuse_bn_bwd_sums = _policy("fuse_bn_bwd", 1) != 0
    fuse_bn_bwd_strided = _policy("fuse_bn_bwd_strided", 1) != 0
    pair_bn_bwd = _policy("pair_bn_bwd", 1) != 0
    fuse_bnwg = _policy("fuse_bnwg", 7)
    pair_ds_sums = _policy("pair_ds_sums", 3)
    z3_free_ds = _policy("z3_free_ds", 1)
    fuse_c3_bwd = _policy("fuse_c3_bwd", 1)
    fuse_mvf_stats = _policy("fuse_mvf_stats", 1) != 0
    dzfree = _policy("dzfree", 2)
    gate_producer = _policy("gate_producer", 1) != 0
    dzfree_q = _policy("dzfree_q", 1)
    dzfree_q_wgs = _policy("dzfree_q_wgs", 256)
    dzfree_q_maxk = _policy("dzfree_q_maxk", 256)
    dzfree_q_mink = _policy("dzfree_q_mink", 0)
    gram_stats = _policy("gram_stats", 1) != 0
    gram_stats_wgs = _policy("gram_stats_wgs", 256)
    gram_colsums = _policy("gram_colsums", 1) != 0

    def side_stream(self):
        if not self.overlap_wgrad:
            return None
        if getattr(self, "_side", None) is None:
            from .streams import concurrent_stream
            self._side = concurrent_stream(self.main_stream())
        return self._side

    def main_stream(self):
        ms = getattr(self, "_main", None)
        return ms if ms is not None else torch.cuda.current_stream()

    _rec = None

    def _wait(self, dst, src):
        if self._rec is not None:
            self._rec.wait(dst, src)
        else:
            dst.wait_stream(src)

    def _mark(self, stream):
        if self._rec is not None:
            return self._rec.mark(stream)
        ev = torch.cuda.Event()
        ev.record(stream)
        return ev

    def _wait_mark(self, stream, ev):
        if self._rec is not None:
            self._rec.wait_mark(stream, ev)
        else:
            stream.wait_event(ev)

    def on_side(self, launch):
        self._side_keep.append(launch)
        self._side_pending.append(launch)


# ... 1426 lines not shown
```

Before: 1852 clips/s.

## Compute strided 1x1 downsample dgrad compactly and scatter it via strided residual epilogues

The downsample branch's stride-2 1x1 conv dgrad now runs as a dense 1x1 conv at the output resolution, producing a compact gradient instead of a full-resolution zero-stuffed one. The following c1 dgrad conv or MVF stencil adds this compact residual through new strided-residual epilogues that map output pixels to compact coordinates and add zero elsewhere. This is meant to remove the wasted work and memory traffic of the zero-filled full-size dgrad. In exchange it adds per-pixel index arithmetic in the epilogues, new template variants, and a gate that is on by default.

```diff
diff --git a/include/mvfnet_hip.h b/include/mvfnet_hip.h
--- a/include/mvfnet_hip.h
+++ b/include/mvfnet_hip.h
@@ -90,6 +90,8 @@
 int mvf_conv2d_nhwc_fwd_resmask_gate_colsums(const mvf_conv_desc_t* d, const void* x, const void* x2, const void* w_packed, const void* residual,
                                              const unsigned char* res_sign_bits, const unsigned char* out_gate_bits, void* y, float* sums_part, void* ws,
                                              size_t ws_bytes, void* stream);
+int mvf_conv2d_nhwc_fwd_sres(const mvf_conv_desc_t* d, const void* x, const void* x2, const void* w_packed, const float* bias, const void* residual,
+                             int res_stride, const unsigned char* out_gate_bits, void* y, float* sums_part, void* ws, size_t ws_bytes, void* stream);
 int mvf_conv2d_nhwc_dgrad_bnsums(const mvf_conv_desc_t* d, const void* dz, const void* w_packed_dgrad, void* y, const void* bn_z,
                                  const float* bn_mean, const float* bn_invstd, const float* bn_scale, const float* bn_shift,
                                  float* sums_part, void* ws, size_t ws_bytes, void* stream);
@@ -360,6 +362,9 @@
 int mvf_nhwc_stencil_gate_colsums(const mvf_desc_t* d, const void* x, int x_c, void* out, int out_c, const float* w_t, const float* w_h,
                                   const float* w_w, int flip, const void* addend, int addend_c, const unsigned char* addend_sign_bits,
                                   const unsigned char* out_gate_bits, float* sums_part, void* stream);
+int mvf_nhwc_stencil_sadd(const mvf_desc_t* d, const void* x, int x_c, void* out, int out_c, const float* w_t, const float* w_h, const float* w_w,
+                          const float* scale, const float* shift, int flip, const void* addend, int addend_c, int addend_stride,
+                          const unsigned char* out_gate_bits, float* sums_part, void* stream);
 int mvf_nhwc_stencil_stats_rows(const mvf_desc_t* d, int x_c, int out_c);
 int mvf_nhwc_stencil_tile_plan(const mvf_desc_t* d, int x_c, int out_c, int* rows_per_band, int* chan_per_wg);
 int mvf_nhwc_stencil_stats(const mvf_desc_t* d, const void* x, int x_c, void* out, int out_c, const float* w_t, const float* w_h,
diff --git a/mvfnet_amd/_lib.py b/mvfnet_amd/_lib.py
--- a/mvfnet_amd/_lib.py
+++ b/mvfnet_amd/_lib.py
@@ -160,6 +160,10 @@
     lib.mvf_conv2d_nhwc_fwd_resmask_gate_colsums.argtypes = [cp, vp, vp, vp, vp, vp, vp, vp, fp, vp, sz, vp]
     lib.mvf_nhwc_stencil_gate_colsums.restype = i32
     lib.mvf_nhwc_stencil_gate_colsums.argtypes = [dp, vp, i32, vp, i32, fp, fp, fp, i32, vp, i32, vp, vp, fp, vp]
+    lib.mvf_conv2d_nhwc_fwd_sres.restype = i32
+    lib.mvf_conv2d_nhwc_fwd_sres.argtypes = [cp, vp, vp, vp, fp, vp, i32, vp, vp, fp, vp, sz, vp]
+    lib.mvf_nhwc_stencil_sadd.restype = i32
+    lib.mvf_nhwc_stencil_sadd.argtypes = [dp, vp, i32, vp, i32, fp, fp, fp, fp, fp, i32, vp, i32, i32, vp, fp, vp]
     lib.mvf_conv2d_nhwc_dgrad_bnsums_split.restype = i32
     lib.mvf_conv2d_nhwc_dgrad_bnsums_split.argtypes = [cp, vp, vp, vp, fp, vp, vp, fp, fp, fp, fp, fp, vp, sz, vp]
     lib.mvf_bn_bwd_dzfree_prep.restype = i32
diff --git a/mvfnet_amd/csrc/conv_nhwc.hip b/mvfnet_amd/csrc/conv_nhwc.hip
--- a/mvfnet_amd/csrc/conv_nhwc.hip
+++ b/mvfnet_amd/csrc/conv_nhwc.hip
@@ -24,6 +24,8 @@
     int N, H, W, Cin, Cout, KH, KW, stride, pad, Ho, Wo;
     int xps, split_c, x2ps, relu;
     int res_c0;
+    int res_s, res_ho, res_wo;
+    unsigned fd_rs_mul, fd_rs_shr;
     const unsigned char* res_mask;
     const unsigned char* out_gate;
     int x_c0;
@@ -844,6 +846,7 @@
     constexpr bool e_apply = EPI == 8;
     const bool e_stats = EPI == 0 ? a.stats_part != nullptr : (EPI == 1 || EPI == 12);
     constexpr bool e_bnb = EPI == 6;
+    constexpr bool e_sres = EPI == 0 || EPI == 3 || EPI == 12;
     const bool e_scatter = (EPI == 0 || EPI == 6) && a.o_s > 0;
     constexpr int CP = BN * 4 + 16;
     constexpr int NH = (LOWK || GLDS) ? 2 : 1;
@@ -894,6 +897,10 @@
         const unsigned nrec = (unsigned)(left < 0x7ffffff0L ? left : 0x7ffffff0L);
         rs_y = __builtin_amdgcn_make_buffer_rsrc((void*)(a.y + base), 0, a.y ? nrec : 0u, 0x00020000);
         rs_res = __builtin_amdgcn_make_buffer_rsrc((void*)(e_res ? a.res + base : (e_bnb ? a.bn_z + base : a.y + base)), 0, nrec, 0x00020000);
+        if (e_sres && a.res_s > 1) {
+            const long rimg = (long)a.res_ho * a.res_wo * a.Cout * ESZ, rleft = (long)(a.N - eimg0) * rimg;
+            rs_res = __builtin_amdgcn_make_buffer_rsrc((void*)(a.res + (long)eimg0 * rimg), 0, (unsigned)(rleft < 0x7ffffff0L ? rleft : 0x7ffffff0L), 0x00020000);
+        }
     }
     const __amdgpu_buffer_rsrc_t rs_mask = __builtin_amdgcn_make_buffer_rsrc(
         (void*)(a.res_mask ? a.res_mask + (long)m0 * (a.Cout / 4) : (const unsigned char*)a.y), 0,
@@ -1087,7 +1094,14 @@
                 }
                 offs[ps] = (cok2 && m < a.M) ? off : kOOB;
                 if (e_res || e_bnb) {
-                    const unsigned roff = (e_bnb || col >= a.res_c0) ? offs[ps] : kOOB;
+                    unsigned roff = (e_bnb || col >= a.res_c0) ? offs[ps] : kOOB;
+                    if (e_sres && a.res_s > 1) {
+                        const int img = fd_div(m, a.fd_hw_mul, a.fd_hw_shr), rem = m - img * (a.Ho * a.Wo);
+                        const int oh = fd_div(rem, a.fd_w_mul, a.fd_w_shr), ow = rem - oh * a.Wo;
+                        const int qh = fd_div(oh, a.fd_rs_mul, a.fd_rs_shr), qw = fd_div(ow, a.fd_rs_mul, a.fd_rs_shr);
+                        const bool on = roff != kOOB && qh * a.res_s == oh && qw * a.res_s == ow;
+                        roff = on ? (unsigned)((((img - eimg0) * a.res_ho + qh) * a.res_wo + qw) * a.Cout + col) * ESZ : kOOB;
+                    }
                     if constexpr (sizeof(ET) == 2) rraw[ps] = __builtin_amdgcn_raw_buffer_load_b64(rs_res, roff, 0, 0);
                     else rraw[ps] = __builtin_amdgcn_raw_buffer_load_b128(rs_res, roff, 0, 0);
                 }
@@ -1283,7 +1297,7 @@
     if (train_like && !a.stats_part && !a.res) return 2;
     if (train_like && !a.stats_part && a.res) return 3;
     if (train_like && a.stats_part && a.res && a.out_gate && !a.bn_z) return 12;
-    if (infer_like(a, epi_spec)) return a.res ? 5 : 4;
+    if (infer_like(a, epi_spec) && a.res_s <= 1) return a.res ? 5 : 4;
     return 0;
 }
 
@@ -1699,7 +1713,7 @@
 static int conv_fwd_impl(const mvf_conv_desc_t* d, const void* x, const void* x2, const void* w_packed, const float* bias,
                          const void* residual, void* y, float* stats_part, const float* stats_shift, void* ws, size_t ws_bytes,
                          void* stream, const unsigned char* res_mask = nullptr, const BnBwdSums* bnb = nullptr, const MvfFuse* mf = nullptr,
-                         const BnApply* ap = nullptr, const BnBwdRecompute* bw = nullptr, const unsigned char* out_gate = nullptr);
+                         const BnApply* ap = nullptr, const BnBwdRecompute* bw = nullptr, const unsigned char* out_gate = nullptr, int res_stride = 0);
 
 int mvf_conv2d_nhwc_fwd_mvf(const mvf_conv_desc_t* d, const void* x, const void* w_packed, const float* bias, const float* mvf_coef,
                             int cs, int n_segment, int act, void* y, void* ws, size_t ws_bytes, void* stream) {
@@ -1779,6 +1793,15 @@
     return conv_fwd_impl(d, x, x2, w_packed, nullptr, residual, y, sums_part, nullptr, ws, ws_bytes, stream, res_sign_bits, nullptr, nullptr, nullptr, nullptr, out_gate_bits);
 }
 
+int mvf_conv2d_nhwc_fwd_sres(const mvf_conv_desc_t* d, const void* x, const void* x2, const void* w_packed, const float* bias, const void* residual,
+                             int res_stride, const unsigned char* out_gate_bits, void* y, float* sums_part, void* ws, size_t ws_bytes, void* stream) {
+    MVF_REQUIRE(d && residual && res_stride >= 1 && d->in_dil <= 1 && (!out_gate_bits || !d->relu) && (!sums_part || (out_gate_bits && !bias)), MVF_EINVAL,
+                "conv2d_sres: needs a residual, res_stride >= 1 and a stride-1 / non-dilated launch; the gate comes without ReLU, the column sums with the gate and without bias");
+    MVF_REQUIRE(!out_gate_bits || (uintptr_t)out_gate_bits % 16 == 0 || d->cout % 64 != 0, MVF_EINVAL, "conv2d_sres: gate byte rows must be 16-byte aligned");
+    return conv_fwd_impl(d, x, x2, w_packed, bias, residual, y, sums_part, nullptr, ws, ws_bytes, stream, nullptr, nullptr, nullptr, nullptr, nullptr, out_gate_bits,
+                         res_stride);
+}
+
 int mvf_conv2d_nhwc_dgrad_bnsums_split(const mvf_conv_desc_t* d, const void* x, const void* x2, const void* w_packed, const float* bias, void* y,
                                        const void* bn_z, const float* bn_mean, const float* bn_invstd, const float* bn_scale, const float* bn_shift,
                                        float* sums_part, void* ws, size_t ws_bytes, void* stream) {
@@ -1817,7 +1840,7 @@
 static int conv_fwd_impl(const mvf_conv_desc_t* d, const void* x, const void* x2, const void* w_packed, const float* bias,
                          const void* residual, void* y, float* stats_part, const float* stats_shift, void* ws, size_t ws_bytes,
                          void* stream, const unsigned char* res_mask, const BnBwdSums* bnb, const MvfFuse* mf, const BnApply* ap, const BnBwdRecompute* bw,
-                         const unsigned char* out_gate) {
+                         const unsigned char* out_gate, int res_stride) {
     t_last_launch = mvf_conv_launch_info_t{};
     MVF_REQUIRE(d && x && w_packed && (y || (stats_part && !bnb)), MVF_EINVAL, "conv2d: NULL argument");
     MVF_REQUIRE(d->dtype == MVF_F32 || d->dtype == MVF_BF16, MVF_EINVAL, "conv2d: bad dtype %d", d->dtype);
@@ -1851,6 +1874,16 @@
     a.res_c0 = d->res_c0 > 0 ? d->res_c0 : 0;
     a.res_mask = res_mask;
     a.out_gate = out_gate;
+    if (res_stride > 1) {
+        MVF_REQUIRE(residual && !res_mask && !bnb && !mf && !ap && !bw && dil == 1 && d->stride == 1 && y, MVF_EINVAL,
+                    "conv2d_sres: a strided residual comes with a plain stride-1 launch (no sign bits, no BatchNorm epilogue)");
+        a.res_s = res_stride;
+        a.res_ho = (d->ho + res_stride - 1) / res_stride;
+        a.res_wo = (d->wo + res_stride - 1) / res_stride;
+        fd_make((unsigned)res_stride, a.fd_rs_mul, a.fd_rs_shr);
+        MVF_REQUIRE((long)a.res_ho * a.res_wo * d->cout * esz * std::min<long>(d->n, 256L / ((long)d->ho * d->wo) + 2) < 0x7ffffff0L, MVF_EUNSUPPORTED,
+                    "conv2d_sres: residual image too large for tile-relative 32-bit addressing");
+    }
     MVF_REQUIRE(d->x_c0 == 0 || (d->split_c > 0 && d->x_c0 > 0 && d->x_c0 <= d->split_c && d->x_c0 % ue == 0 && d->x_pix_stride >= d->cin - d->x_c0), MVF_EINVAL,
                 "conv2d: x_c0=%d needs a split operand (split_c=%d), 0 < x_c0 <= split_c, a multiple of %d, and x rows of >= cin - x_c0 channels", d->x_c0, d->split_c, ue);
     a.x_c0 = d->x_c0;
diff --git a/mvfnet_amd/csrc/mvf_nhwc.hip b/mvfnet_amd/csrc/mvf_nhwc.hip
--- a/mvfnet_amd/csrc/mvf_nhwc.hip
+++ b/mvfnet_amd/csrc/mvf_nhwc.hip
@@ -34,7 +34,15 @@
     unsigned fdw_mul, fdw_shr, fdrw_mul, fdrw_shr;
     const float* stats_shift;
     const unsigned char* out_gate;
+    int add_s, add_ho, add_wo;
 };
+
+__device__ __forceinline__ int addend_pixel(const NhwcArgs& a, int h, int w) {
+    if (a.add_s <= 1) return h * a.w + w;
+    const int qh = h / a.add_s, qw = w / a.add_s;
+    return (qh * a.add_s == h && qw * a.add_s == w) ? qh * a.add_wo + qw : -1;
+}
+__device__ __forceinline__ int addend_frame(const NhwcArgs& a) { return a.add_s <= 1 ? a.h * a.w : a.add_ho * a.add_wo; }
 
 __device__ __forceinline__ float tap3(float w0, float w1, float w2, float a, float b, float c) { return __builtin_fmaf(w2, c, __builtin_fmaf(w1, b, w0 * a)); }
 
@@ -120,10 +128,16 @@
             }
             if (a.add) {
                 float ad[VEC];
-                const long apix = ((long)n * T + t) * HW + pix;
-                Vec<ET, VEC>::load(reinterpret_cast<const ET*>(a.add) + apix * a.add_c + c0, ad);
+                const int ap0 = addend_pixel(a, hh, wv);
+                const long apix = ((long)n * T + t) * addend_frame(a) + ap0;
                 unsigned mb = 0xfu;
-                if (a.add_mask) mb = a.add_mask[apix * (a.add_c / 4) + c0 / 4] >> (c0 & 3);
+                if (ap0 >= 0) {
+                    Vec<ET, VEC>::load(reinterpret_cast<const ET*>(a.add) + apix * a.add_c + c0, ad);
+                    if (a.add_mask) mb = a.add_mask[apix * (a.add_c / 4) + c0 / 4] >> (c0 & 3);
+                } else {
+#pragma unroll
+                    for (int i = 0; i < VEC; ++i) ad[i] = 0.f;
+                }
 #pragma unroll
                 for (int i = 0; i < VEC; ++i) y[i] += ((mb >> i) & 1u) ? ad[i] : 0.f;
             }
@@ -142,7 +156,7 @@
     }
 }
 
-template <typename ET, int TB>
+template <typename ET, int TB, bool SADD = false>
 __global__ __launch_bounds__(kThreads) void mvf_nhwc_apply_chunked(NhwcArgs a) {
     constexpr int VEC = 4;
     const int HW = a.h * a.w, W = a.w, H = a.h, T = a.T, C = a.c;
@@ -199,6 +213,7 @@
         const long o0 = ((long)n * T * HW + pix) * a.out_c + c0;
         const bool ok_up = vh && hh > 0, ok_dn = vh && hh < H - 1, ok_lf = vw && wv > 0, ok_rt = vw && wv < W - 1;
         const long d_up = ok_up ? -(long)W * C : 0, d_dn = ok_dn ? (long)W * C : 0, d_lf = ok_lf ? -(long)C : 0, d_rt = ok_rt ? (long)C : 0;
+        const int ap0 = SADD ? addend_pixel(a, hh, wv) : pix, aHW = SADD ? addend_frame(a) : HW;
         for (int t0 = 0; t0 < T; t0 += TB) {
             float cen[TB + 2][VEC], up[TB][VEC], dn[TB][VEC], lf[TB][VEC], rt[TB][VEC], ad[TB][VEC];
             unsigned mb[TB], gb[TB];
@@ -219,10 +234,13 @@
                 mb[k] = 0xfu;
                 gb[k] = 0xfu;
                 if (a.out_gate) gb[k] = a.out_gate[(((long)n * T + t) * HW + pix) * (a.out_c / 4) + c0 / 4] >> (c0 & 3);
-                if (a.add) {
-                    const long apix = ((long)n * T + t) * HW + pix;
+                if (a.add && (!SADD || ap0 >= 0)) {
+                    const long apix = ((long)n * T + t) * aHW + ap0;
                     Vec<ET, VEC>::load(reinterpret_cast<const ET*>(a.add) + apix * a.add_c + c0, ad[k]);
                     if (a.add_mask) mb[k] = a.add_mask[apix * (a.add_c / 4) + c0 / 4] >> (c0 & 3);
+                } else if (SADD) {
+#pragma unroll
+                    for (int i = 0; i < VEC; ++i) ad[k][i] = 0.f;
                 }
             }
 #pragma unroll
@@ -290,7 +308,7 @@
     shr = l;
 }
 
-template <int TT, int CW>
+template <int TT, int CW, bool SADD = false>
 __global__ __launch_bounds__(kThreads, 2) void mvf_nhwc_apply_lds(NhwcArgs a) {
     extern __shared__ __attribute__((aligned(16))) char lds_tile[];
     constexpr int VEC = 4, NG = CW / VEC, PPT = CW / 8;
@@ -365,6 +383,7 @@
         const long pix0 = (long)n * TT * HW + h * W + w;
         constexpr int TC = 4;
         struct Side { uint2 ad[TC]; unsigned mb[TC], gb[TC]; };
+        const int ap0 = SADD ? addend_pixel(a, h, w) : 0, aHW = SADD ? addend_frame(a) : 0;
         auto load_side = [&](int tc, Side& sd) {
 #pragma unroll
             for (int k = 0; k < TC; ++k) {
@@ -372,9 +391,10 @@
                 sd.mb[k] = 0xfu;
                 sd.gb[k] = 0xfu;
                 sd.ad[k] = make_uint2(0u, 0u);
-                if (a.add) {
-                    sd.ad[k] = *reinterpret_cast<const uint2*>(reinterpret_cast<const bf16_t*>(a.add) + apix * a.add_c + c0);
-                    if (a.add_mask) sd.mb[k] = a.add_mask[apix * (a.add_c / 4) + c0 / 4];
+                if (a.add && ap0 >= 0) {
+                    const long qpix = SADD ? ((long)n * TT + tc + k) * aHW + ap0 : apix;
+                    sd.ad[k] = *reinterpret_cast<const uint2*>(reinterpret_cast<const bf16_t*>(a.add) + qpix * a.add_c + c0);
+                    if (a.add_mask) sd.mb[k] = a.add_mask[qpix * (a.add_c / 4) + c0 / 4];
                 }
                 if (a.out_gate) sd.gb[k] = a.out_gate[apix * (a.out_c / 4) + c0 / 4];
             }
@@ -491,6 +511,12 @@
 template <int TT>
 static void launch_lds(const NhwcArgs& a, const LdsPlan& p, hipStream_t st) {
     dim3 grid(a.n_clips * p.bands, a.cs / p.cw);
+    if (a.add_s > 1) {
+        if (p.cw == 64) hipLaunchKernelGGL((mvf_nhwc_apply_lds<TT, 64, true>), grid, dim3(kThreads), p.lds, st, a);
+        else if (p.cw == 32) hipLaunchKernelGGL((mvf_nhwc_apply_lds<TT, 32, true>), grid, dim3(kThreads), p.lds, st, a);
+        else hipLaunchKernelGGL((mvf_nhwc_apply_lds<TT, 16, true>), grid, dim3(kThreads), p.lds, st, a);
+        return;
+    }
     if (p.cw == 64) hipLaunchKernelGGL((mvf_nhwc_apply_lds<TT, 64>), grid, dim3(kThreads), p.lds, st, a);
     else if (p.cw == 32) hipLaunchKernelGGL((mvf_nhwc_apply_lds<TT, 32>), grid, dim3(kThreads), p.lds, st, a);
     else hipLaunchKernelGGL((mvf_nhwc_apply_lds<TT, 16>), grid, dim3(kThreads), p.lds, st, a);
@@ -509,7 +535,7 @@
 
 }
 
-struct NhwcFlip { int flip; const void* add; int add_c; const unsigned char* add_mask; const unsigned char* out_gate; float* stats_part; const float* stats_shift; int rows_only; };
+struct NhwcFlip { int flip; const void* add; int add_c; const unsigned char* add_mask; const unsigned char* out_gate; float* stats_part; const float* stats_shift; int rows_only; int add_s; };
 int mvf_nhwc_fwd_infer_impl2(const mvf_desc_t* d, const void* x, void* out, int out_c, const float* wt, const float* wh,
                              const float* ww, const float* scale, const float* shift, NhwcFlip fl, hipStream_t st) {
     if (!fl.rows_only) t_last_stencil = mvf_stencil_launch_info_t{};
@@ -526,6 +552,11 @@
     a.add_c = fl.add_c;
     a.add_mask = fl.add_mask;
     a.out_gate = fl.out_gate;
+    if (fl.add && fl.add_s > 1) {
+        a.add_s = fl.add_s;
+        a.add_ho = (d->h + fl.add_s - 1) / fl.add_s;
+        a.add_wo = (d->w + fl.add_s - 1) / fl.add_s;
+    }
     a.stats_part = fl.stats_part;
     a.stats_shift = fl.stats_shift;
     const int esz = d->dtype == MVF_F32 ? 4 : 2;
@@ -581,11 +612,13 @@
     t_last_stencil = rec;
     if (use_lds) {
     } else if (d->dtype == MVF_F32) {
-        if (chunked) hipLaunchKernelGGL((mvf_nhwc_apply_chunked<float, 4>), grid, dim3(kThreads), 0, st, a);
+        if (chunked && a.add_s > 1) hipLaunchKernelGGL((mvf_nhwc_apply_chunked<float, 4, true>), grid, dim3(kThreads), 0, st, a);
+        else if (chunked) hipLaunchKernelGGL((mvf_nhwc_apply_chunked<float, 4>), grid, dim3(kThreads), 0, st, a);
         else if (vec) hipLaunchKernelGGL((mvf_nhwc_apply<float, 4>), grid, dim3(kThreads), 0, st, a);
         else hipLaunchKernelGGL((mvf_nhwc_apply<float, 1>), grid, dim3(kThreads), 0, st, a);
     } else {
-        if (chunked) hipLaunchKernelGGL((mvf_nhwc_apply_chunked<bf16_t, 8>), grid, dim3(kThreads), 0, st, a);
+        if (chunked && a.add_s > 1) hipLaunchKernelGGL((mvf_nhwc_apply_chunked<bf16_t, 8, true>), grid, dim3(kThreads), 0, st, a);
+        else if (chunked) hipLaunchKernelGGL((mvf_nhwc_apply_chunked<bf16_t, 8>), grid, dim3(kThreads), 0, st, a);
         else if (vec) hipLaunchKernelGGL((mvf_nhwc_apply<bf16_t, 4>), grid, dim3(kThreads), 0, st, a);
         else hipLaunchKernelGGL((mvf_nhwc_apply<bf16_t, 1>), grid, dim3(kThreads), 0, st, a);
     }
@@ -929,6 +962,19 @@
     return mvf_nhwc_fwd_infer_impl2(&dd, x, out, out_c, w_t, w_h, w_w, scale, shift, f, (hipStream_t)stream);
 }
 
+int mvf_nhwc_stencil_sadd(const mvf_desc_t* d, const void* x, int x_c, void* out, int out_c, const float* w_t, const float* w_h, const float* w_w,
+                          const float* scale, const float* shift, int flip, const void* addend, int addend_c, int addend_stride,
+                          const unsigned char* out_gate_bits, float* sums_part, void* stream) {
+    t_last_stencil = mvf_stencil_launch_info_t{};
+    MVF_REQUIRE(d && x && out && w_t && x != out && x_c >= d->cs && out_c >= d->cs && addend && addend_stride >= 1, MVF_EINVAL, "nhwc_stencil_sadd: bad argument");
+    MVF_REQUIRE(addend_c >= d->cs, MVF_EINVAL, "nhwc_stencil_sadd: addend pitch < cs");
+    MVF_REQUIRE(!sums_part || (out_gate_bits && !scale && !shift), MVF_EINVAL, "nhwc_stencil_sadd: the column sums come with the output gate and without the activation");
+    mvf_desc_t dd = *d;
+    dd.c = x_c;
+    NhwcFlip f = {flip, addend, addend_c, nullptr, out_gate_bits, sums_part, nullptr, 0, addend_stride};
+    return mvf_nhwc_fwd_infer_impl2(&dd, x, out, out_c, w_t, w_h, w_w, scale, shift, f, (hipStream_t)stream);
+}
+
 int mvf_nhwc_stencil_gate_colsums(const mvf_desc_t* d, const void* x, int x_c, void* out, int out_c, const float* w_t, const float* w_h,
                                   const float* w_w, int flip, const void* addend, int addend_c, const unsigned char* addend_sign_bits,
                                   const unsigned char* out_gate_bits, float* sums_part, void* stream) {
diff --git a/mvfnet_amd/train_engine.py b/mvfnet_amd/train_engine.py
--- a/mvfnet_amd/train_engine.py
+++ b/mvfnet_amd/train_engine.py
@@ -214,6 +214,13 @@
         return dz
 
 
+class _StridedRes(object):
+    __slots__ = ("t", "s")
+
+    def __init__(self, t, s):
+        self.t, self.s = t, s
+
+
 class _TConv(object):
 
     def __init__(self, conv, eng, stem=False):
@@ -223,6 +230,7 @@
         self.cout, self.cin, self.kh, self.kw = conv.weight.shape
         self.stride, self.pad = conv.stride[0], conv.padding[0]
         self.stem = stem
+        self.compact = False
         dev = conv.weight.device
         td = eng.tdtype
         if stem:
@@ -401,10 +409,27 @@
                                                _p(part), _p(ws), ws.numel(), _st()), "conv dgrad+bn sums")
 
     def dgrad(self, dz, n, ho, wo, h, w, residual=None, res_c0=0, res_bits=None, out_gate=None, gsum=None):
+        ws = _conv_ws(dz.device)
+        if self.compact and self.stride > 1 and self.kh == 1 and self.kw == 1 and self.pad == 0 and residual is None and out_gate is None:
+            d = ConvDesc(n, ho, wo, self.cout, self.cin, 1, 1, 1, 0, ho, wo, self.cout, self.eng.dt, 0, 0, 0, 0, 0)
+            dxc = self.eng.buf((id(self), "dx_compact"), (n * ho * wo, self.cin))
+            check(lib.mvf_conv2d_nhwc_fwd_resmask(C.byref(d), _p(dz), None, _p(self.wd), None, None, None, _p(dxc), _p(ws), ws.numel(), _st()), "conv dgrad (compact)")
+            return _StridedRes(dxc, self.stride)
         d = ConvDesc(n, ho, wo, self.cout, self.cin, self.kh, self.kw, 1, self.kh - 1 - self.pad, h, w, self.cout, self.eng.dt, 0, 0, 0,
                      self.stride if self.stride > 1 else 0, res_c0)
         dx = self.eng.buf((id(self), "dx"), (n * h * w, self.cin))
-        ws = _conv_ws(dz.device)
+        if isinstance(residual, _StridedRes):
+            assert res_bits is None
+            part = rows = None
+            if out_gate is not None and gsum is not None:
+                bn = gsum["bn"]
+                rows = _stats_rows(d)
+                part = self.eng.buf((id(bn), "gsum_conv"), (self.cin, rows, 2), torch.float32)
+            check(lib.mvf_conv2d_nhwc_fwd_sres(C.byref(d), _p(dz), None, _p(self.wd), None, _p(residual.t), residual.s, _p(out_gate), _p(dx), _p(part), _p(ws),
+                                               ws.numel(), _st()), "conv dgrad (strided residual)")
+            if part is not None:
+                bn._s1 = [None, 0, res_c0, part, rows]
+            return dx
         if out_gate is not None and gsum is not None:
             bn = gsum["bn"]
             rows = _stats_rows(d)
@@ -580,6 +605,18 @@
         self.launch_stencil(d, dy, self.cs, dxp, c, 1, addend, c if addend is not None else 0, addend_bits, out_gate, gsum)
 
     def launch_stencil(self, d, src, src_c, dst, dst_c, flip, addend, addend_c, addend_bits, out_gate=None, gsum=None):
+        if isinstance(addend, _StridedRes):
+            assert addend_bits is None
+            part = None
+            if out_gate is not None and gsum is not None:
+                bn = gsum["bn"]
+                rows = lib.mvf_nhwc_stencil_stats_rows(C.byref(d), src_c, dst_c)
+                part = self.eng.buf((id(bn), "gsum_mvf"), (self.cs, rows, 2), torch.float32)
+            check(lib.mvf_nhwc_stencil_sadd(C.byref(d), _p(src), src_c, _p(dst), dst_c, _p(self.wt), _p(self.wh), _p(self.ww), None, None, flip, _p(addend.t),
+                                            addend_c, addend.s, _p(out_gate), _p(part), _st()), "mvf stencil (strided addend)")
+            if part is not None:
+                bn._s1[0], bn._s1[1] = part, rows
+            return
         if out_gate is not None and gsum is not None:
             bn = gsum["bn"]
             rows = lib.mvf_nhwc_stencil_stats_rows(C.byref(d), src_c, dst_c)
@@ -826,6 +863,7 @@
         elif self.cd is not None:
             if dzd is None:
                 dzd = self.bd.backward(g, self.cd.cout, s["zd"], m2, eng, 4, ymask=bits)
+            self.cd.compact = bool(eng.strided_dgrad) and (self.mvf is None or self.mvf.cs % 4 == 0)
             resid, rbits = self.cd.dgrad(dzd, nt, ho, wo, h, w), None
             if not wd_done:
                 self.cd.wgrad(dzd, s["x"], nt, h, w, ho, wo, eng, x_pitch=c)
@@ -989,6 +1027,7 @@
     fuse_bn_bwd_sums = _policy("fuse_bn_bwd", 1) != 0
     fuse_bn_bwd_strided = _policy("fuse_bn_bwd_strided", 1) != 0
     pair_bn_bwd = _policy("pair_bn_bwd", 1) != 0
+    strided_dgrad = _policy("strided_dgrad", 1) != 0
     fuse_bnwg = _policy("fuse_bnwg", 7)
     pair_ds_sums = _policy("pair_ds_sums", 3)
     z3_free_ds = _policy("z3_free_ds", 1)
```

Result: no change. 1867 clips/s, median of 6 (+0.8%).
